# cgmb/euler

Measured on AMD Instinct MI355X. Metric: cells*steps/sec of sim_step() (frames incl. the PCG pressure projection) + pressure-solve HBM GB/s vs roofline, higher is better.
Workload: dtype f64

## Files before the change

### euler_amd/__init__.py

```python
import ctypes as C
import os

import numpy as np

_HERE = os.path.dirname(os.path.abspath(__file__))
LIB_PATH = os.path.join(_HERE, "lib", "libeuler_hip.so")

DOT_AUTO, DOT_SEQUENTIAL, DOT_TREE = 0, 1, 2
PRECOND_IC0, PRECOND_JACOBI, PRECOND_IC0_TILE, PRECOND_IC0_TILE2, PRECOND_IC0_TILE_MG = 0, 1, 2, 3, 4
(OPT_P_STEPS, OPT_TILE_STORE_AS, OPT_TILE_REVERSE, OPT_RESIDENT_CAP, OPT_GRID4_MIN_CELLS, OPT_SLAB_FUSION, OPT_RCCL_SMALL, OPT_RCCL_NO_EXCHANGE, OPT_MARKERS_ROWMAJOR,
 OPT_SA_RUN, OPT_NO_INTERIOR, OPT_BUILD_GATHER, OPT_RESIDENT_FORCE_TIMEOUT, OPT_MG_SPLIT_LEVEL, OPT_MG_SPLIT_ACTIVE, OPT_MARKERS_TWO_PASS, OPT_BUILD_TWO_PASS,
 OPT_VELOCITY_TWO_PASS, OPT_NO_TILE_MAP, OPT_PROFILE_STRIDE, OPT_TILE_STORE_Z, OPT_ADVECT_RK2, OPT_ADVECT_MACCORMACK) = range(1, 24)
SWEEP_AUTO, SWEEP_BAND, SWEEP_SIMPLE = 0, 1, 2
PCG_F64, PCG_F32 = 0, 1
RESIDENT_AUTO, RESIDENT_OFF = 0, 1
IMAGE_COVERAGE, IMAGE_DYE, IMAGE_SPEED = 0, 1, 2
EDIT_SOLID, EDIT_CLEAR, EDIT_SINK, EDIT_SOURCE, EDIT_FILL, EDIT_DRAIN = range(6)
OVERVIEW_DTYPE = np.dtype({"names": ["cells", "solid", "sink", "water", "marks", "max_speed2", "dye"],
                           "formats": [np.uint32, np.uint32, np.uint32, np.uint32, np.uint32, np.float32, (np.uint64, 3)],
                           "offsets": [0, 4, 8, 12, 16, 20, 24], "itemsize": 48})
DIAG_CROWDED = 8
DIAG_DTYPE = np.dtype({"names": ["cells", "fluid", "markers", "crowded", "mass_x", "mass_y", "div_l1", "ke_hi", "ke_lo", "count_max", "nonfinite", "max_div", "max_speed2"],
                       "formats": [np.uint64] * 9 + [np.uint32, np.uint32, np.float32, np.float32],
                       "offsets": [0, 8, 16, 24, 32, 40, 48, 56, 64, 72, 76, 80, 84], "itemsize": 88})
FLOW_PRESSURE = 1
PAINT_VORTICITY, PAINT_PRESSURE, PAINT_SPEED = 0, 1, 2
FLOW_DTYPE = np.dtype({"names": ["cells", "water", "nodes", "nonfinite", "u_pos", "u_neg", "v_pos", "v_neg", "w_pos", "w_neg", "p_sum", "max_speed2", "max_abs_w", "max_p", "reserved"],
                       "formats": [np.uint32] * 4 + [np.uint64] * 7 + [np.float32] * 3 + [np.uint32],
                       "offsets": [0, 4, 8, 12, 16, 24, 32, 40, 48, 56, 64, 72, 76, 80, 84], "itemsize": 88})
GAUGE_LEVEL, GAUGE_PRESSURE, GAUGE_FORCE, GAUGE_FLUX = range(4)
GAUGES_MAX = 1024
GAUGE_DTYPE = np.dtype({"names": ["kind", "x0", "y0", "x1", "y1", "reserved"], "formats": [np.int32] * 6, "offsets": [0, 4, 8, 12, 16, 20], "itemsize": 24})
GAUGE_REC_DTYPE = np.dtype({"names": ["cells", "fluid", "lo_x", "hi_x", "lo_y", "hi_y", "terms", "nonfinite", "a_pos", "a_neg", "b_pos", "b_neg", "max_a", "max_b"],
                            "formats": [np.uint32] * 8 + [np.uint64] * 4 + [np.float32] * 2,
                            "offsets": [0, 4, 8, 12, 16, 20, 24, 28, 32, 40, 48, 56, 64, 68], "itemsize": 72})
FORCE_BOXES_MAX = 64
FORCING_DTYPE = np.dtype({"names": ["gx", "gy", "shake_x", "shake_y", "shake_hz", "shake_phase", "nboxes", "reserved", "reserved2"],
                          "formats": [np.float32] * 4 + [np.float64] * 2 + [np.int32] * 2 + [np.float64],
                          "offsets": [0, 4, 8, 12, 16, 24, 32, 36, 40], "itemsize": 48})
FORCE_BOX_DTYPE = np.dtype({"names": ["x0", "y0", "x1", "y1", "fx", "fy"], "formats": [np.int32] * 4 + [np.float32] * 2, "offsets": [0, 4, 8, 12, 16, 20], "itemsize": 24})
HEAT_BOXES_MAX = 64
HEAT_FIX, HEAT_RATE = 0, 1
HEAT_DTYPE = np.dtype({"names": ["ambient", "beta", "kappa", "source_t", "nboxes", "reserved", "reserved2"],
                       "formats": [np.float32] * 4 + [np.int32] * 2 + [np.float64], "offsets": [0, 4, 8, 12, 16, 20, 24], "itemsize": 32})
HEAT_PX_DTYPE = np.dtype({"names": ["cells", "water", "t_pos", "t_neg", "max_above", "max_below"], "formats": [np.uint32] * 2 + [np.uint64] * 2 + [np.float32] * 2,
                          "offsets": [0, 4, 8, 16, 24, 28], "itemsize": 32})
HEAT_BOX_DTYPE = np.dtype({"names": ["x0", "y0", "x1", "y1", "value", "kind"], "formats": [np.int32] * 4 + [np.float32, np.int32], "offsets": [0, 4, 8, 12, 16, 20], "itemsize": 24})
BODIES_MAX = 16
BODY_DTYPE = np.dtype({"names": ["x", "y", "hz", "phase", "vx", "vy", "amp_x", "amp_y", "w", "h", "reserved"],
                       "formats": [np.float64] * 4 + [np.float32] * 4 + [np.int32] * 2 + [(np.int32, 2)],
                       "offsets": [0, 8, 16, 24, 32, 36, 40, 44, 48, 52, 56], "itemsize": 64})
BODY_STATE_DTYPE = np.dtype({"names": ["px", "py", "ox", "oy"], "formats": [np.float64] * 2 + [np.int32] * 2, "offsets": [0, 8, 16, 20], "itemsize": 24})
RESEED_DTYPE = np.dtype({"names": ["thin_above", "fill_holes", "max_cells", "max_fill", "reserved"], "formats": [np.int32] * 4 + [(np.int32, 4)],
                         "offsets": [0, 4, 8, 12, 16], "itemsize": 32})
RESEED_STATS_DTYPE = np.dtype({"names": ["removed", "added", "cells_thinned", "deferred"], "formats": [np.uint64] * 4, "offsets": [0, 8, 16, 24], "itemsize": 32})
ENV_ARRIVAL, ENV_WET, ENV_SPEED, ENV_PRESSURE, ENV_ALL = 1, 2, 4, 8, 15
ENV_NAMES = {ENV_ARRIVAL: "arrival", ENV_WET: "wet", ENV_SPEED: "speed", ENV_PRESSURE: "pressure"}
ENVELOPE_PX_DTYPE = np.dtype({"names": ["cells", "touched", "arrival_min", "arrival_max", "wet_max", "speed2_max", "p_max", "reserved"],
                              "formats": [np.uint32] * 8, "offsets": [0, 4, 8, 12, 16, 20, 24, 28], "itemsize": 32})
TRACERS_MAX = 1 << 22
TRACER_WET, TRACER_RETIRED, TRACER_IN_SOLID, TRACER_IN_SINK, TRACER_LOST, TRACER_WAS_DRY = 1, 2, 4, 8, 16, 32
TRACER_RASTER_ALL = 1
TRACER_DTYPE = np.dtype({"names": ["x", "y", "path", "age", "wet_time", "substeps", "flags", "reserved"],
                         "formats": [np.float32] * 5 + [np.uint32] * 3, "offsets": [0, 4, 8, 12, 16, 20, 24, 28], "itemsize": 32})
SESSION_IGNORE_SETTINGS = 1
SESSION_OPTS = 32
SESSION_SETTINGS_DTYPE = np.dtype({"names": ["max_iterations", "dot_mode", "precond", "tile_records", "sweep_mode", "max_substeps", "rainbow", "pcg_precision", "resident",
                                             "pcg_poll_interval", "viscosity_bits", "frame_time_bits", "tol", "nopts", "reserved", "opt"],
                                   "formats": [np.int32] * 10 + [np.uint32] * 2 + [np.float64] + [np.int32] * 2 + [(np.int64, SESSION_OPTS)],
                                   "offsets": [0, 4, 8, 12, 16, 20, 24, 28, 32, 36, 40, 44, 48, 56, 60, 64], "itemsize": 320})
SESSION_STAT_KEYS = ("last_substeps", "last_pcg_iterations", "last_residual", "last_dt", "pad", "marker_dt_events", "marker_multi_events")
SESSION_STAT_FORMAT = "<iidfIQQ"
SESSION_TAGS = (b"TIME", b"FORC", b"HEAT", b"TRAC", b"BODY", b"RSED", b"SETT", b"STAT", b"END\0")
GAUGE_VALUES = ("a", "b", "mean_a", "depth")
DIAG_VALUES = ("mean_abs_div", "kinetic_energy", "com_x", "com_y", "markers_per_cell", "crowded_fraction")
(F_U, F_V, F_UTMP, F_VTMP, F_SOLID, F_SOURCE, F_SINK, F_COUNT, F_PREV_COUNT, F_MARKERS, F_PRECON,
 F_PRESSURE, F_PCG_B, F_PCG_R, F_PCG_Z, F_PCG_S, F_PCG_Q, F_CELLMASK,
 F_DYE_R, F_DYE_G, F_DYE_B, F_DYE_RTMP, F_DYE_GTMP, F_DYE_BTMP, F_MARKER_KEYS) = range(25)
(STAGE_ADVECT_MARKERS, STAGE_REFRESH_COUNTS, STAGE_SOURCES, STAGE_EXTRAPOLATE, STAGE_ADVECT_VELOCITY,
 STAGE_PROJECT) = range(6)
(OP_BUILD_SYSTEM, OP_PRECON_FACTOR, OP_FORWARD_SOLVE, OP_BACKWARD_SOLVE, OP_APPLY_A, OP_DOT_ZR, OP_DOT_ZS,
 OP_INF_NORM_R, OP_UPDATE_PR, OP_UPDATE_SEARCH) = range(10)

_FIELD_DTYPE = {
    F_U: np.float32, F_V: np.float32, F_UTMP: np.float32, F_VTMP: np.float32,
    F_SOLID: np.uint8, F_SOURCE: np.uint8, F_SINK: np.uint8, F_COUNT: np.uint8, F_PREV_COUNT: np.uint8,
    F_MARKERS: np.float32, F_PRECON: np.float64, F_PRESSURE: np.float64, F_PCG_B: np.float64,
    F_PCG_R: np.float64, F_PCG_Z: np.float64, F_PCG_S: np.float64, F_PCG_Q: np.float64, F_CELLMASK: np.uint8,
    F_DYE_R: np.float32, F_DYE_G: np.float32, F_DYE_B: np.float32,
    F_DYE_RTMP: np.float32, F_DYE_GTMP: np.float32, F_DYE_BTMP: np.float32, F_MARKER_KEYS: np.uint32,
}


class EulerError(RuntimeError):
    def __init__(self, code, msg):
# ... 996 lines not shown
```

### euler_amd/csrc/driver.hip

```cpp
#include "euler_dev.h"
#include "k_mg.h"

#include <math.h>
#include <stdarg.h>
#include <stdlib.h>
#include <string.h>

#include <vector>

int eu_launch_build_system(euler_sim* S, float dt);
int eu_launch_velocity_update(euler_sim* S, float dt, int finish);
int eu_pressure_current(euler_sim* S);
int eu_unskew(euler_sim* S, const void* skew, void* rowmajor, int elem_bytes);
int eu_unskew_fluid(euler_sim* S, const double* skew, double* rowmajor);
double* eu_current_search_direction(euler_sim* S);
int eu_launch_tile_table(euler_sim* S);
int eu_skew(euler_sim* S, const void* rowmajor, void* skew, int elem_bytes);
int eu_set_source_count(euler_sim* S, size_t nsrc);

static thread_local char g_err[512] = "";

void eu_set_error(const char* fmt, ...) {
  va_list ap;
  va_start(ap, fmt);
// ... 56 lines not shown
}

extern "C" int euler_profile_class_count(void) { return KC__COUNT; }
extern "C" const char* euler_profile_class_name(int32_t c) { return (c >= 0 && c < KC__COUNT) ? k_class_names[c] : ""; }
extern "C" int euler_profile_enable(euler_sim* S, uint64_t mask) {
  if (!S) return EULER_EINVAL;
  int rc = eu_prof_flush(S);
  S->prof_mask = mask;
  S->prof_open = 0;
  return rc;
}
extern "C" int euler_profile_get(euler_sim* S, int32_t cls, double* ms, uint64_t* launches) {
  if (!S || cls < 0 || cls >= KC__COUNT) return EULER_EINVAL;
  int rc = eu_prof_flush(S);
  if (ms) *ms = S->prof_ms[cls];
  if (launches) *launches = S->prof_launches[cls];
  return rc;
}
extern "C" int euler_profile_reset(euler_sim* S) {
  if (!S) return EULER_EINVAL;
  int rc = eu_prof_flush(S);
  memset(S->prof_ms, 0, sizeof(S->prof_ms));
  memset(S->prof_launches, 0, sizeof(S->prof_launches));
  memset(S->prof_idle, 0, sizeof(S->prof_idle));
  return rc;
}

extern "C" int euler_config_default(euler_config* c) {
  if (!c) return EULER_EINVAL;
  memset(c, 0, sizeof(*c));
  c->abi_version = EULER_ABI_VERSION;
  c->X = 100; c->Y = 40;
  c->device = 0;
  c->max_iterations = 100;
  c->tol = (double)1e-6f;
  c->dot_mode = EULER_DOT_AUTO;
  c->precond = EULER_PRECOND_IC0;
  c->sweep_mode = EULER_SWEEP_AUTO;
  c->max_substeps = 8;
  c->frame_time = 0.1f;
  c->viscosity = 0.f;
  c->pcg_poll_interval = 8;
  return EULER_OK;
}

static int eu_set_tiles(euler_sim* S, int w) {
  if (w <= 0) w = 16;
  if (w != 8 && w != 16 && w != 32) { eu_set_error("precond_tile_records = %d: 8, 16 or 32 (0 = 16)", w); return EULER_EINVAL; }
  S->cfg.precond_tile_records = w;
  S->tile_w = w;
  return EULER_OK;
}

bool eu_resident_eligible(const euler_sim* S) {
  if (S->res_disabled || S->cfg.resident == EULER_RESIDENT_OFF) return false;
  if (S->cfg.precond != EULER_PRECOND_IC0_TILE || S->tile_w != 16 || S->cfg.sweep_mode == EULER_SWEEP_SIMPLE || S->cfg.dot_mode != EULER_DOT_TREE) return false;
  if (S->has_comm || S->slab_on || S->p2p_on) return false;
  const int cap = eu_resident_capacity(const_cast<euler_sim*>(S), S->cfg.pcg_precision == EULER_PCG_F32);
  if (S->cfg.pcg_precision == EULER_PCG_F32) return cap > 0 && S->geom.nbands * (S->geom.T / 16) <= 4 * cap;
  return cap > 0;
}
extern "C" int euler_resident_info(euler_sim* S, uint64_t out[3]) {
  if (!S || !out) return EULER_EINVAL;
  out[0] = eu_resident_eligible(S) ? 1 : 0; out[1] = S->res_solves; out[2] = S->res_fallbacks;
  return EULER_OK;
}

extern "C" int euler_set_option(euler_sim* S, int32_t key, int64_t value) {
  if (!S || key <= 0 || key >= EULER_OPT__COUNT) { eu_set_error("euler_set_option: unknown key %d", (int)key); return EULER_EINVAL; }
  bool ok = true;
  const char* when = nullptr;
  switch (key) {
    case EULER_OPT_P_STEPS: ok = value == 2 || value == 4 || value == 8; break;
    case EULER_OPT_SA_RUN: ok = value == 8 || value == 16 || value == 32;
      if (ok && value != 8 && (S->has_comm || eu_is_two_level(S))) when = "on a handle without a communicator, in the parity or the plain tile-local mode (the others run runs of 8)";
      break;
    case EULER_OPT_RCCL_SMALL: ok = value >= 0 && value <= 2; if (S->rccl) when = "before euler_set_comm_rccl"; break;
    case EULER_OPT_RCCL_NO_EXCHANGE: ok = value == 0 || value == 1; if (S->rccl) when = "before euler_set_comm_rccl"; break;
    case EULER_OPT_SLAB_FUSION: ok = value == 0 || value == 1; if (S->p2p_on) when = "before euler_p2p_connect"; break;
    case EULER_OPT_RESIDENT_CAP: case EULER_OPT_GRID4_MIN_CELLS: case EULER_OPT_RESIDENT_FORCE_TIMEOUT: ok = value >= 0; break;
    case EULER_OPT_MG_SPLIT_LEVEL: ok = value >= -1 && value < 12; break;
    case EULER_OPT_PROFILE_STRIDE: ok = value >= 1 && value <= 1024; break;
    case EULER_OPT_MG_SPLIT_ACTIVE: ok = false; break;
    case EULER_OPT_ADVECT_RK2: ok = value == 0 || value == 1;
      if (ok && value == 1 && S->slab_on) when = "on a whole-grid handle (row slabs: the midpoint samples reach one row beyond the ghost rows)";
      break;
    case EULER_OPT_ADVECT_MACCORMACK: ok = value == 0 || value == 1;
      if (ok && value == 1 && S->slab_on) when = "on a whole-grid handle (row slabs: the correction reads the forward result one row beyond the own rows)";
      break;
    default: ok = value == 0 || value == 1; break;
  }
  if (!ok) { eu_set_error("euler_set_option: key %d does not take the value %lld", (int)key, (long long)value); return EULER_EINVAL; }
  if (when) { eu_set_error("euler_set_option: key %d must be set %s", (int)key, when); return EULER_ESTATE; }
  HIPCHK(hipStreamSynchronize(S->stream));
  if (key == EULER_OPT_ADVECT_MACCORMACK && value == 1 && !S->mc_u) {
    float *a = nullptr, *b = nullptr;
    const size_t bytes = S->C * sizeof(float);
    if (eu_dalloc(S, &a, S->C, EU_MEM_HANDLE, EU_MEM_ZERO | EU_DEV_QUIET) || eu_dalloc(S, &b, S->C, EU_MEM_HANDLE, EU_MEM_ZERO | EU_DEV_QUIET)) {
      (void)eu_dev_free(S, a);
      eu_set_error("euler_set_option: EULER_OPT_ADVECT_MACCORMACK needs %zu bytes of scratch", 2 * bytes);
      return EULER_ENOMEM;
    }
    S->mc_u = a; S->mc_v = b;
  }
  if (key == EULER_OPT_P_STEPS || key == EULER_OPT_SA_RUN) {
    int rcp = eu_pressure_current(S);
    if (rcp) return rcp;
  }
  S->opt[key] = value;
  if (key == EULER_OPT_P_STEPS || key == EULER_OPT_SA_RUN) S->s_ring_n = 0;
  if (key == EULER_OPT_MG_SPLIT_LEVEL) { eu_mg_split_release(S); S->opt[EULER_OPT_MG_SPLIT_ACTIVE] = 0; }
  return EULER_OK;
}
extern "C" int euler_get_option(euler_sim* S, int32_t key, int64_t* value) {
  if (!S || !value || key <= 0 || key >= EULER_OPT__COUNT) { eu_set_error("euler_get_option: unknown key %d", (int)key); return EULER_EINVAL; }
  *value = S->opt[key];
  return EULER_OK;
}

static const char* eu_precond_combination(const euler_sim* S, int precond, int tile_w, int has_comm, int slab_on, int p2p_on) {
  const bool coarse = precond == EULER_PRECOND_IC0_TILE2 || precond == EULER_PRECOND_IC0_TILE_MG;
  if (!coarse) return nullptr;
  if (tile_w != 16 || S->cfg.sweep_mode == EULER_SWEEP_SIMPLE) return "the coarse-correction preconditioners run on tiles of 16 records with the band schedule";
  if (precond == EULER_PRECOND_IC0_TILE2 && (has_comm || slab_on)) return "EULER_PRECOND_IC0_TILE2 runs on one GPU (row slabs: EULER_PRECOND_IC0_TILE_MG)";
  if (precond == EULER_PRECOND_IC0_TILE_MG && has_comm && (!slab_on || p2p_on)) return "EULER_PRECOND_IC0_TILE_MG with several ranks: row-slab handles without mailboxes only";
  return nullptr;
}

extern "C" int euler_set_precond(euler_sim* S, int32_t precond, int32_t tile_records) {
  if (!S || precond < EULER_PRECOND_IC0 || precond > EULER_PRECOND_IC0_TILE_MG) { eu_set_error("euler_set_precond: bad argument"); return EULER_EINVAL; }
  const int w = tile_records <= 0 ? 16 : tile_records;
  if (w != 8 && w != 16 && w != 32) { eu_set_error("precond_tile_records = %d: 8, 16 or 32 (0 = 16)", tile_records); return EULER_EINVAL; }
  if (const char* why = eu_precond_combination(S, precond, w, S->has_comm, S->slab_on, S->p2p_on)) { eu_set_error("euler_set_precond: %s", why); return EULER_EINVAL; }
  if (S->cfg.pcg_precision == EULER_PCG_F32 && (precond != EULER_PRECOND_IC0_TILE || w != 16)) { eu_set_error("euler_set_precond: an EULER_PCG_F32 handle runs EULER_PRECOND_IC0_TILE with tiles of 16 records only"); return EULER_EINVAL; }
  HIPCHK(hipStreamSynchronize(S->stream));
  const bool coarse = precond == EULER_PRECOND_IC0_TILE2 || precond == EULER_PRECOND_IC0_TILE_MG;
  if (coarse) { int rc = eu_coarse_alloc(S, precond == EULER_PRECOND_IC0_TILE_MG); if (rc) return rc; }
  (void)eu_set_tiles(S, w);
  S->cfg.dot_mode = coarse ? EULER_DOT_TREE : S->dot_mode_user;
  if (S->has_comm && S->cfg.dot_mode == EULER_DOT_SEQUENTIAL) S->cfg.dot_mode = EULER_DOT_TREE;
  S->cfg.precond = precond;
  eu_vd_solver_arrays_foreign(&S->vd);
  return EULER_OK;
}

extern "C" int euler_set_solver(euler_sim* S, int32_t max_iterations, double tol) {
  if (!S) return EULER_EINVAL;
  HIPCHK(hipStreamSynchronize(S->stream));
  if (max_iterations > 0) S->cfg.max_iterations = max_iterations;
  if (tol >= 0.0) S->cfg.tol = tol;
  return EULER_OK;
}

#define DALLOC(p, n) do { int _rc = eu_dalloc(S, &(p), (n), EU_MEM_HANDLE, EU_MEM_ZERO); if (_rc) { euler_destroy(S); return _rc; } } while (0)

extern "C" void euler_destroy(euler_sim* S) {
  if (!S) return;
  if (S->stream) (void)hipStreamSynchronize(S->stream);
  eu_p2p_release(S);
  eu_rccl_release(S);
  eu_slab_release(S);
  eu_coarse_release(S);
  eu_dev_free_all(S);
  if (S->ms_host) (void)hipHostFree(S->ms_host);
  if (S->sc_host) (void)hipHostFree(S->sc_host);
  if (S->poll_host) (void)hipHostFree(S->poll_host);
// ... 849 lines not shown
```

### euler_amd/csrc/euler_dev.h

```cpp
#pragma once

#include <hip/hip_runtime.h>
#include <stdint.h>
#include <stdio.h>

#include "euler.h"
#include "euler_host.h"
#include "eu_valid.h"
#include "eu_mem.h"

#define EU_H 1.0f
#define EU_RHO 1.0f
#define EU_G (-10.0f)

#define CM_FLUID 0x01
#define CM_RIGHT 0x02
#define CM_UP    0x04
#define CM_LEFT  0x08
#define CM_DOWN  0x10
#define CM_DIAG_SHIFT 5
#define CM_INTERIOR 0x9F
#define EU_CHUNK_INTERIOR 0x80000000u

enum {
  KC_TIMESTEP = 0, KC_MARKER_ADVECT, KC_MARKER_EVENTS, KC_MARKER_BIN, KC_MARKER_COMPACT, KC_SOURCES,
  KC_SELECT, KC_EXTRAPOLATE, KC_ADVECT_VELOCITY, KC_BUILD_SYSTEM, KC_PRECON_FACTOR,
  KC_FORWARD_SOLVE, KC_BACKWARD_SOLVE, KC_APPLY_A, KC_DOT, KC_UPDATE_PR, KC_UPDATE_SEARCH,
  KC_REDUCE_FINAL, KC_VELOCITY_UPDATE, KC_JACOBI, KC_MISC, KC_PRECOND_TILE, KC_COARSE_CYCLE, KC_RESIDENT, KC__COUNT
};

struct PcgScalars {
  double sigma, zs, sigma_new, alpha, beta, rnorm;
  double tol;
  double comm_val;
  double comm_val2;
  double* comm_slot;
  double alpha_prev;
  double alpha_hist[8];
  int nonzero;
  int done;
  int iters;
  int max_iters;
  unsigned int n_chunks;
  unsigned int zfix;
  void** p2p_boxes;
  int* p2p_error;
  int p2p_rank, p2p_n;
  unsigned int p2p_seq, p2p_halo_seq;
};

struct MarkerState {
  unsigned long long n;
  unsigned long long max_markers;
  unsigned long long rng_state;
  int exhausted;
  unsigned int n_events;
  unsigned int n_actual;
  unsigned int n_deleted;
  unsigned int n_append;
  unsigned long long n0_append;
  unsigned long long total_dt_events, multi_events;
  float dt_final;
  float dt;
  unsigned int max_u2_bits, max_v2_bits;
  unsigned int dt_ticket;
  int error;
  unsigned long long n_loc;
  unsigned int n_rm;
  unsigned int n_del_glob;
  unsigned int n_recv;
  unsigned int src_k_lo;
  unsigned long long rng0;
  unsigned int rs_crowded;
  unsigned int rs_k;
  unsigned int rs_holes;
  unsigned int rs_fill;
  unsigned long long rs_n0;
  unsigned long long rs_rng0;
  unsigned long long rs_removed, rs_added, rs_thinned, rs_deferred;
};

#define EU_SKEW_SLACK (64 * 64)
#ifndef EU_ARRAY_STAGGER
#define EU_ARRAY_STAGGER 0
#endif
#ifndef EU_RED_ELEMS
#define EU_RED_ELEMS (256 * 16)
#endif
struct SkewGeom {
  int X, Y, nbands, T, TS;
  size_t S;
};
static inline __host__ __device__ size_t skew_index(const SkewGeom& g, int x, int y) {
  const int l = y & 63, t = x + l;
  return ((size_t)(y >> 6) * g.TS + (size_t)(t & ~1)) * 64 + 2 * l + (t & 1);
}
static inline __host__ __device__ void skew_decode(const SkewGeom& g, size_t e, int& band, int& t, int& l) {
  const size_t per_band = (size_t)g.TS * 64;
  band = (int)(e / per_band);
  const size_t r = e % per_band;
  l = (int)((r & 127) >> 1);
  t = (int)((r >> 7) << 1) + (int)(r & 1);
}

struct SelectScratch {
  unsigned int* block_sums;
  unsigned int* total;
  size_t capacity_blocks;
};

struct eu_devbuf { void* p; size_t bytes; };

struct euler_sim {
  euler_config cfg;
  int X, Y;
  size_t C;
  hipStream_t stream;
  int loaded;
  long long opt[32];
  int dot_mode_user;

  float *u, *v, *utmp, *vtmp;
  uint8_t *solid, *source, *sink, *count, *prev_count;
  unsigned int* count32;
  eu_valid vd;
  unsigned long long* delmask;
  uint8_t* tmap;
// ... 13 lines not shown
  size_t n_tracers;
  euler_heat heat;
  euler_heat_box heat_boxes[EULER_HEAT_BOXES_MAX];
  int heat_on, heat_cur;
  int heat_ghost_stale;
  unsigned int heat_ntiles;
  eu_devbuf heat_buf, heat_box_buf, heat_fill_buf, heat_ras_buf;
  int n_bodies;
  euler_body bodies[EULER_BODIES_MAX];
  int32_t body_ox[EULER_BODIES_MAX], body_oy[EULER_BODIES_MAX];
  euler_reseed reseed;
  int reseed_on;
  eu_devbuf rs_mask_buf, rs_cell_buf, rs_slot_buf, rs_draw_buf;
  uint32_t env_channels;
  uint64_t env_substeps;
  uint32_t* env_plane[4];
  eu_devbuf env_ras_buf;
  float *mc_u, *mc_v;
  float2* markers[2];
  int cur;
  size_t max_markers;
  unsigned long long n_markers_host;
  size_t n_source_cells;
  MarkerState* ms;
  MarkerState* ms_host;
  unsigned long long* evmask;
  float* ev_theta;
  float* ev_delta;
  unsigned int* sel_idx;
  size_t sel_cap;
  unsigned int* act_idx; float* act_dt;
  unsigned long long* cellmask64;
  float* draws;
  SelectScratch sel;

  SkewGeom geom;
  double *b, *p, *r, *z, *s, *q, *precon;
  double* s2;
  uint8_t* cellmask;
  uint8_t* sys_m; float* sys_div;
  unsigned int* fbits_fwd; unsigned int* fbits_bwd;
  int fb_stride;
  int4* band_ranges;
  int coarse_m, coarse_shift, coarse_nx, coarse_ny, coarse_n;
  int *cc_diag, *cc_right, *cc_up;
  int* cc_pinned;
  double* cc_sten;
  int cc_n;
  double* cc_fac;
  double* cc_inv;
  double* cc_part;
  double* cc_y;
  double* cc_null;
  int mg_levels, mg_nx[12], mg_ny[12];
  size_t mg_off[12], mg_cells;
  double* mg_a;
  unsigned long long* mg_a0i;
  double *mg_rhs, *mg_x;
  double* mg_wd;
  uint8_t* mg_inner0; double mg_ic[9];
  double* mg_part;
  double* mg_dot;
  double* mg_null0;
  double* mg_m0;
  void* mg_split;
  double* mg_xbuf; int mg_xslot;
  unsigned long long* res_gran;
  unsigned long long res_tag;
  int* res_err;
  int res_disabled;
  unsigned int res_last_chunks;
  int res_have_last, res_skip_once;
  unsigned long long res_solves, res_fallbacks;
  int pcg_fields_resident;
  int tile_w;
  double* s_ring[8];
  void* s_ring_alloc[8];
  double* s_base[2];
  int s_ring_n;
  int s_launched;
  int s_none;
  int s_stale;
  const double* tile_as_override;
  double* partial2;
  struct RngJump* rng_jump;
  uint8_t* chunk_flag;
  uint8_t* chunk_prev;
  uint8_t* chunk_part;
  eu_mem mem;
  double* zhalo;
  double* zrows;
  int z_halo_last;
  double* tile_table;
  unsigned long long* chunk_bits;
  unsigned int* chunk_list;
  size_t chunk_words, chunk_cap;
  double* xrows;
  size_t xrow_len;
  int gs_cur;
  double* alpha_buf;
  double* pair_buf;
  double* rowmajor_tmp;
  PcgScalars* sc;
  PcgScalars* sc_host;
  PcgScalars* poll_host;
  hipEvent_t poll_event[2];
  double* partial;
  unsigned int* red_counter;
  int red_blocks;
  unsigned long long* granules;
  int gran_stride;
  unsigned int* ticket;
  unsigned int ticket_base;
  unsigned int epoch;
  unsigned long long* sweep_timeline;

  float interp_lim[4];

  euler_stats stats;

  euler_comm_ops comm;
  int has_comm, couple;
  int band_lo, band_hi;
  size_t e_lo, e_cnt;
  double* halo_buf;
  int own_stream;
  int slab_on;
  int row_lo, row_hi, win_lo, win_hi;
  size_t win_off, Cw, skew_off, Sw;
  int ab_lo, ab_hi;
  unsigned int* keys[2];
  euler_comm_ops bulk;
  struct SlabScratch* slab;
  int part_lo[64], part_hi[64];
  void* rccl;
  void* p2p;
  int p2p_on;

  uint64_t prof_mask;
  uint64_t prof_open;
  unsigned int prof_seq[32];
  double prof_ms[KC__COUNT];
  uint64_t prof_launches[KC__COUNT];
  uint64_t prof_idle[KC__COUNT];
  hipEvent_t* ev_pool; int* ev_cls; int* ev_solve; int* ev_iter; int ev_used, ev_cap;
  int solve_seq;
  int prof_iter;
  int solve_iters[256];
};

void eu_set_error(const char* fmt, ...);
int eu_hip_fail(hipError_t e, const char* what, const char* file, int line);
#define HIPCHK(call) do { hipError_t _e = (call); if (_e != hipSuccess) return eu_hip_fail(_e, #call, __FILE__, __LINE__); } while (0)

void eu_prof_begin(euler_sim* S, int cls);
void eu_prof_end(euler_sim* S, int cls);
int  eu_prof_flush(euler_sim* S);

#define LAUNCH(S, CLS, KERNEL, GRID, BLOCK, ...)                                   \
  do {                                                                             \
    eu_prof_begin((S), (CLS));                                                     \
    hipLaunchKernelGGL(KERNEL, GRID, BLOCK, 0, (S)->stream, __VA_ARGS__);          \
    eu_prof_end((S), (CLS));                                                       \
  } while (0)

static inline unsigned eu_blocks(size_t n, unsigned per_block, unsigned cap = 0x7fffffffu) {
  size_t b = (n + per_block - 1) / per_block;
  if (b < 1) b = 1;
  if (b > cap) b = cap;
  return (unsigned)b;
}

__device__ __forceinline__ size_t eu_xcd_block() {
  const unsigned int b = blockIdx.x, full = gridDim.x & ~7u;
  return b < full ? (size_t)(b & 7) * (full >> 3) + (b >> 3) : (size_t)b;
// ... 236 lines not shown
```

### euler_amd/csrc/k_grid.hip

```cpp
#include "k_pcg.h"
#include "k_transport.h"

#include <stdlib.h>

__device__ __forceinline__ void dt_from_maxima(MarkerState* ms, float frame_time_left, unsigned int mu_bits, unsigned int mv_bits) {
  const float mu = __uint_as_float(mu_bits), mv = __uint_as_float(mv_bits);
  const float max_distance = 0.75f * EU_H;
  const float max_velocity = sqrtf(mu + mv);
  ms->dt = fminf(max_distance / max_velocity, frame_time_left);
  ms->max_u2_bits = 0u;
  ms->max_v2_bits = 0u;
}
template <bool FUSE_DT>
__global__ __launch_bounds__(256) void k_maxsq(const float* __restrict__ u, const float* __restrict__ v,
                                               int X, int Y, MarkerState* ms, int y0, int y1, float frame_time_left) {
  float mu = 0.f, mv = 0.f;
  const bool vec = (X & 3) == 0;
  for (int yq = y0 + 4 * (int)blockIdx.x; yq < y1; yq += 4 * (int)gridDim.x) {
    if (vec) {
      for (int x = 4 * (int)threadIdx.x; x < X; x += 4 * 256) {
        float4 a[4], b[4];
#pragma unroll
        for (int r = 0; r < 4; ++r) {
          const int y = yq + r < y1 ? yq + r : y1 - 1;
// ... 591 lines not shown
      sm[ll[k]][jj[k]] = mm[k];
      sd[ll[k]][jj[k]] = dv[k];
      if (mm[k] & CM_FLUID) s_fl[jj[k] / 16] = 1;
      if (mm[k] != CM_INTERIOR) s_part[jj[k] / 16] = 1;
    }
  }
  __syncthreads();
  const float k_inv_scale_f = (EU_H * EU_H) * EU_RHO / dt;
  bool nz = false;
  for (int c = tid; c < 64 * BS_W; c += 256) {
    const int pr = c >> 7, l = (c & 127) >> 1, j = 2 * pr + (c & 1);
    const int ch = j / 16;
    const bool touch = s_fl[ch] || s_prev[ch];
    const int x = t0 + j - l, y = band * 64 + l;
    if (!touch || x < 0 || x >= X || y >= Y) continue;
    const uint8_t m = sm[l][j];
    const double bv = m ? -(double)sd[l][j] * (double)k_inv_scale_f : 0.0;
    nz = nz || bv != 0.0;
    const size_t e = ((size_t)band * g.TS + (size_t)(t0 + 2 * pr)) * 64 + (size_t)(c & 127);
    cellmask[e] = m;
    b[e] = bv;
    r[e] = bv;
    p[e] = 0.0;
    if (!TILE) { q[e] = 0.0; z[e] = 0.0; }
  }
  if (nz) s_nz = 1;
  __syncthreads();
  if (tid < BS_W / 16) {
    if (s_fl[tid]) chunk_flag[chunk0 + tid] = 1;
    if (s_part[tid]) chunk_part[chunk0 + tid] = 1;
  }
  if (tid == 0 && s_nz && __hip_atomic_load(&sc->nonzero, __ATOMIC_RELAXED, __HIP_MEMORY_SCOPE_AGENT) == 0) atomicOr(&sc->nonzero, 1);
}

__global__ __launch_bounds__(256) void k_pack_chunk_bits(const uint8_t* __restrict__ flag, unsigned long long* __restrict__ bits, size_t nwords, size_t nchunks) {
  const size_t w = (size_t)blockIdx.x * blockDim.x + threadIdx.x;
  if (w >= nwords) return;
  unsigned long long v = 0;
  for (int k = 0; k < 64; ++k) {
    const size_t c = w * 64 + k;
    if (c < nchunks && flag[c]) v |= 1ull << k;
  }
  bits[w] = v;
}

__global__ __launch_bounds__(256) void k_velocity_update(const float* __restrict__ uin, const float* __restrict__ vin,
                                                         float* __restrict__ uout, float* __restrict__ vout,
                                                         double* p, const uint8_t* __restrict__ count,
                                                         const uint8_t* __restrict__ solid, SkewGeom g, float dt, int y0, int y1) {
  const int X = g.X, Y = g.Y;
  const int x = blockIdx.x * 64 + (threadIdx.x & 63);
  const int y = y0 + blockIdx.y * 4 + (threadIdx.x >> 6);
  if (x >= X || y >= y1) return;
  const size_t i = (size_t)y * X + x;
  const size_t e = skew_index(g, x, y);
  const bool f0 = count[i] != 0;
  double p0 = p[e];
  if (f0 && p0 < 0.0) { p0 = 0.0; p[e] = 0.0; }
  const float neg_inv = -(1.f / (EU_RHO * EU_H));
  if (x < X - 1) {
    const bool f1 = count[i + 1] != 0;
    float o = 0.f;
    if (solid[i] | solid[i + 1]) o = 0.f;
    else if (f0 | f1) {
      double p1 = p[skew_index(g, x + 1, y)];
      if (f1 && p1 < 0.0) p1 = 0.0;
      o = uin[i] + (neg_inv * (float)(p1 - p0)) * dt;
    }
    uout[i] = o;
  }
  if (y < Y - 1) {
    const bool f1 = count[i + X] != 0;
    float o = 0.f;
    if (solid[i] | solid[i + X]) o = 0.f;
    else if (f0 | f1) {
      double p1 = p[skew_index(g, x, y + 1)];
      if (f1 && p1 < 0.0) p1 = 0.0;
      o = vin[i] + (neg_inv * (float)(p1 - p0)) * dt;
    }
    vout[i] = o;
  }
}

struct VuRing { const double* s[8]; int n, steps, use; };
#define VU_W 48
#define VU_ILP 4
__global__ __launch_bounds__(256) void k_velocity_update_para(const float* __restrict__ uin, const float* __restrict__ vin, float* __restrict__ uout, float* __restrict__ vout,
                                                              const double* __restrict__ p, const uint8_t* __restrict__ mask, const uint8_t* __restrict__ count,
                                                              const uint8_t* __restrict__ solid, SkewGeom g, float dt, const PcgScalars* sc, VuRing ring, MarkerState* ms,
                                                              int band_lo, int do_max, int skip_zero,
                                                              const uint8_t* __restrict__ tmap, int tnx) {
  __shared__ double sp[65][VU_W + 1];
  __shared__ float s_mu[4], s_mv[4];
  const int units = g.T / VU_W;
  const size_t blk = eu_xcd_block();
  const int band = band_lo + (int)(blk / units), t0 = (int)(blk % units) * VU_W;
  const int X = g.X, Y = g.Y, tid = threadIdx.x;
  if (skip_zero && tmap && eu_tiles_idle_cur(tmap, tnx, band, t0 > 63 ? (t0 - 63) >> 6 : 0, (t0 + VU_W - 1) >> 6, true)) return;
  int cnt = 0, from = 0;
  if (ring.use && sc->nonzero && sc->iters > 0) {
    const int n_it = sc->iters;
    from = n_it - 1 >= ring.steps ? (n_it - 1) / ring.steps * ring.steps : 0;
    cnt = n_it - from;
  }
  double al[8];
  const double* sq[8];
#pragma unroll
  for (int j = 0; j < 8; ++j) { const int it = from + (j < cnt ? j : 0); al[j] = sc->alpha_hist[it & 7]; sq[j] = ring.s[it % ring.n]; }
  const size_t ebase = ((size_t)band * g.TS + (size_t)t0) * 64;
  static_assert((64 * VU_W) % (256 * VU_ILP) == 0, "whole rounds of VU_ILP elements per thread");
  for (int c0 = tid; c0 < 64 * VU_W; c0 += 256 * VU_ILP) {
    uint8_t m[VU_ILP];
    double pv[VU_ILP];
    bool any = false;
#pragma unroll
    for (int u = 0; u < VU_ILP; ++u) { m[u] = mask[ebase + (size_t)(c0 + 256 * u)]; any = any || (m[u] & CM_FLUID); }
    if (__any(any)) {
#pragma unroll
      for (int u = 0; u < VU_ILP; ++u) pv[u] = p[ebase + (size_t)(c0 + 256 * u)];
#pragma unroll
      for (int j = 0; j < 8; ++j)
        if (j < cnt) {
          double sv[VU_ILP];
#pragma unroll
          for (int u = 0; u < VU_ILP; ++u) sv[u] = sq[j][ebase + (size_t)(c0 + 256 * u)];
#pragma unroll
          for (int u = 0; u < VU_ILP; ++u) pv[u] = pv[u] + sv[u] * al[j];
        }
    } else {
#pragma unroll
      for (int u = 0; u < VU_ILP; ++u) pv[u] = 0.0;
    }
#pragma unroll
    for (int u = 0; u < VU_ILP; ++u) {
      const int c = c0 + 256 * u;
      const double v = (m[u] & CM_FLUID) ? (pv[u] < 0.0 ? 0.0 : pv[u]) : 0.0;
      sp[(c & 127) >> 1][2 * (c >> 7) + (c & 1)] = v;
    }
  }
  {
    size_t e = 0;
    bool want = false, above = false;
    int hl = 0, hj = 0;
    if (tid < 64) { e = ebase + (size_t)VU_W * 64 + 2 * (size_t)tid; want = true; hl = tid; hj = VU_W; }
    else if (tid < 64 + VU_W) {
      const int j = tid - 64 + 1, x = t0 - 64 + j;
      hl = 64; hj = j;
      if (x >= 0 && x < X && band + 1 < g.nbands && count[(size_t)(band + 1) * 64 * X + x] != 0) { e = ((size_t)(band + 1) * g.TS + (size_t)(x & ~1)) * 64 + (size_t)(x & 1); want = true; above = true; }
    }
    if (tid < 64 + VU_W) {
      double pv = 0.0;
      if (want && (above || (mask[e] & CM_FLUID))) {
        pv = p[e];
#pragma unroll
        for (int j = 0; j < 8; ++j) if (j < cnt) pv = pv + sq[j][e] * al[j];
        pv = pv < 0.0 ? 0.0 : pv;
      }
      sp[hl][hj] = pv;
    }
  }
  __syncthreads();
  const float neg_inv = -(1.f / (EU_RHO * EU_H));
  float mu = 0.f, mv = 0.f;
  static_assert((64 * VU_W) % (256 * 4) == 0, "whole rounds of four cells per thread");
  for (int c0 = tid; c0 < 64 * VU_W; c0 += 256 * 4) {
    size_t ii[4]; bool in[4]; int ll[4], jj[4], xx[4], yy[4];
    uint8_t c_0[4], c_r[4], c_u[4], s_0[4], s_r[4], s_u[4];
    float ui[4], vi[4];
#pragma unroll
    for (int u = 0; u < 4; ++u) {
      const int c = c0 + 256 * u;
      ll[u] = c / VU_W; jj[u] = c % VU_W;
      xx[u] = t0 - ll[u] + jj[u]; yy[u] = band * 64 + ll[u];
      in[u] = xx[u] >= 0 && xx[u] < X && yy[u] < Y;
      ii[u] = (size_t)(yy[u] < Y ? yy[u] : Y - 1) * X + (size_t)(xx[u] < 0 ? 0 : xx[u] >= X ? X - 1 : xx[u]);
      const bool hr = in[u] && xx[u] < X - 1, hu = in[u] && yy[u] < Y - 1;
      c_0[u] = count[ii[u]]; s_0[u] = solid[ii[u]];
      c_r[u] = count[ii[u] + (hr ? 1 : 0)]; s_r[u] = solid[ii[u] + (hr ? 1 : 0)];
      c_u[u] = count[ii[u] + (hu ? (size_t)X : (size_t)0)]; s_u[u] = solid[ii[u] + (hu ? (size_t)X : (size_t)0)];
    }
    bool wet = false;
#pragma unroll
    for (int u = 0; u < 4; ++u) wet = wet || ((c_0[u] | c_r[u] | c_u[u]) != 0);
    if (__any(wet)) {
#pragma unroll
      for (int u = 0; u < 4; ++u) { ui[u] = uin[ii[u]]; vi[u] = vin[ii[u]]; }
// ... 23 lines not shown
        if (s_0[u] | s_u[u]) o = 0.f;
        else if (f0 | f1) { o = vi[u] + (neg_inv * (float)(sp[l + 1][j + 1] - p0)) * dt; live = true; }
        if (live || !skip_zero) vout[ii[u]] = o;
        const float sqv = o * o; if (sqv > mv) mv = sqv;
      }
    }
  }
  mu = eu_wave_maxf(mu);
  mv = eu_wave_maxf(mv);
  if ((tid & 63) == 0) { s_mu[tid >> 6] = mu; s_mv[tid >> 6] = mv; }
  __syncthreads();
  if (tid == 0 && do_max) {
    for (int k = 1; k < 4; ++k) { if (s_mu[k] > mu) mu = s_mu[k]; if (s_mv[k] > mv) mv = s_mv[k]; }
    if (mu > 0.f) atomicMax(&ms->max_u2_bits, __float_as_uint(mu));
    if (mv > 0.f) atomicMax(&ms->max_v2_bits, __float_as_uint(mv));
  }
}
__global__ __launch_bounds__(256) void k_clamp_p(double* __restrict__ p, const uint8_t* __restrict__ mask, size_t e_lo, size_t S) {
  for (size_t i = e_lo + (size_t)blockIdx.x * blockDim.x + threadIdx.x; i < e_lo + S; i += (size_t)gridDim.x * blockDim.x)
    if ((mask[i] & CM_FLUID) && p[i] < 0.0) p[i] = 0.0;
}

__global__ __launch_bounds__(256) void k_mark_interior(unsigned int* __restrict__ list, const PcgScalars* sc, const uint8_t* __restrict__ part) {
  const unsigned int i = blockIdx.x * blockDim.x + threadIdx.x;
  if (i >= sc->n_chunks) return;
  const unsigned int c = list[i];
  if (!part[c]) list[i] = c | EU_CHUNK_INTERIOR;
}

int eu_launch_build_system(euler_sim* S, float dt) {
  uint8_t* t = S->chunk_flag; S->chunk_flag = S->chunk_prev; S->chunk_prev = t;
  HIPCHK(hipMemsetAsync(S->chunk_flag, 0, S->chunk_cap + 64, S->stream));
  HIPCHK(hipMemsetAsync(S->chunk_part, 0, S->chunk_cap + 64, S->stream));
  const bool lean = eu_vd_lean_assembly(&S->vd, eu_is_tile(S) && S->cfg.sweep_mode != EULER_SWEEP_SIMPLE);
  const bool gather = S->opt[EULER_OPT_BUILD_GATHER] != 0;
  const bool two_pass = S->opt[EULER_OPT_BUILD_TWO_PASS] != 0;
  if (!gather && !two_pass) {
    const unsigned nblk = (unsigned)((size_t)(S->band_hi - S->band_lo) * (S->geom.T / BS_W));
    if (lean)
      LAUNCH(S, KC_BUILD_SYSTEM, k_build_system_para<true>, dim3(nblk), dim3(256), S->utmp, S->vtmp, S->count, S->solid, S->b, S->r, S->p, S->q, S->z, S->cellmask, S->sc, S->geom, dt, S->band_lo,
             S->chunk_flag, S->chunk_part, S->chunk_prev, eu_tile_map_on(S) ? (const uint8_t*)S->tmap : (const uint8_t*)nullptr, S->tmap_nx);
    else
      LAUNCH(S, KC_BUILD_SYSTEM, k_build_system_para<false>, dim3(nblk), dim3(256), S->utmp, S->vtmp, S->count, S->solid, S->b, S->r, S->p, S->q, S->z, S->cellmask, S->sc, S->geom, dt, S->band_lo,
             S->chunk_flag, S->chunk_part, S->chunk_prev, (const uint8_t*)nullptr, 0);
  } else if (!gather) {
    const size_t win_off = (size_t)S->win_lo * S->X;
    LAUNCH(S, KC_BUILD_SYSTEM, k_cell_system, dim3(eu_blocks((size_t)S->X * (S->row_hi - S->row_lo), 256)), dim3(256), S->utmp, S->vtmp, S->count, S->solid, S->sys_m, S->sys_div,
           S->X, S->row_lo, S->row_hi, win_off);
    if (lean)
      LAUNCH(S, KC_BUILD_SYSTEM, k_build_system2<true>, dim3(eu_blocks(S->e_cnt, 256)), dim3(256), S->sys_m, S->sys_div, win_off, S->b, S->r, S->p, S->q, S->z, S->cellmask, S->sc,
             S->geom, dt, S->e_lo, S->e_cnt, S->chunk_flag, S->chunk_part, S->chunk_prev);
    else
      LAUNCH(S, KC_BUILD_SYSTEM, k_build_system2<false>, dim3(eu_blocks(S->e_cnt, 256)), dim3(256), S->sys_m, S->sys_div, win_off, S->b, S->r, S->p, S->q, S->z, S->cellmask, S->sc,
             S->geom, dt, S->e_lo, S->e_cnt, S->chunk_flag, S->chunk_part, S->chunk_prev);
  } else if (lean)
    LAUNCH(S, KC_BUILD_SYSTEM, k_build_system<true>, dim3(eu_blocks(S->e_cnt, 256)), dim3(256), S->utmp, S->vtmp, S->count,
           S->solid, S->b, S->r, S->p, S->q, S->z, S->cellmask, S->sc, S->geom, dt, S->e_lo, S->e_cnt, S->chunk_flag, S->chunk_part, S->chunk_prev);
  else
    LAUNCH(S, KC_BUILD_SYSTEM, k_build_system<false>, dim3(eu_blocks(S->e_cnt, 256)), dim3(256), S->utmp, S->vtmp, S->count,
           S->solid, S->b, S->r, S->p, S->q, S->z, S->cellmask, S->sc, S->geom, dt, S->e_lo, S->e_cnt, S->chunk_flag, S->chunk_part, S->chunk_prev);
  eu_vd_assembled(&S->vd);
  LAUNCH(S, KC_BUILD_SYSTEM, k_pack_chunk_bits, dim3(eu_blocks(S->chunk_words, 256)), dim3(256), S->chunk_flag, S->chunk_bits, S->chunk_words, S->chunk_cap);
  int rc = eu_ordered_select(S, S->chunk_bits, S->chunk_words, S->chunk_list, &S->sc->n_chunks);
  if (rc) return rc;
  const bool no_interior = S->opt[EULER_OPT_NO_INTERIOR] != 0;
  if (!no_interior)
    LAUNCH(S, KC_BUILD_SYSTEM, k_mark_interior, dim3(eu_blocks(S->chunk_cap, 256)), dim3(256), S->chunk_list, S->sc, S->chunk_part);
  return eu_launch_band_ranges(S);
}

int eu_pressure_current(euler_sim* S) {
  const int mode = eu_vd_pressure_owes(&S->vd);
  if (!mode) return EULER_OK;
  eu_vd_pressure_made_current(&S->vd);
  if (mode == 1) { int rc = eu_launch_finish_p(S); if (rc) return rc; }
  LAUNCH(S, KC_VELOCITY_UPDATE, k_clamp_p, dim3(eu_blocks(S->e_cnt, 256 * 4, 4096)), dim3(256), S->p, S->cellmask, S->e_lo, S->e_cnt);
  return EULER_OK;
}
int eu_launch_velocity_update(euler_sim* S, float dt, int finish) {
  const bool one_pass = (!S->has_comm || S->slab_on) && S->opt[EULER_OPT_VELOCITY_TWO_PASS] == 0 && (!S->slab_on || !finish);
  if (one_pass) {
    VuRing ring;
    for (int k = 0; k < 8; ++k) ring.s[k] = S->s_ring[k < S->s_ring_n ? k : 0];
    ring.n = S->s_ring_n > 0 ? S->s_ring_n : 1; ring.steps = ring.n; ring.use = finish && S->s_ring_n > 0;
    if (!ring.use) for (int k = 0; k < 8; ++k) ring.s[k] = S->p;
    const int do_max = S->slab_on ? 0 : 1;
    if (eu_vd_update_clears_maxima(&S->vd, do_max)) HIPCHK(hipMemsetAsync(&S->ms->max_u2_bits, 0, 2 * sizeof(unsigned int), S->stream));
    LAUNCH(S, KC_VELOCITY_UPDATE, k_velocity_update_para, dim3((unsigned)((size_t)(S->band_hi - S->band_lo) * (S->geom.T / VU_W))), dim3(256), S->utmp, S->vtmp, S->u, S->v, S->p, S->cellmask,
           S->count, S->solid, S->geom, dt, S->sc, ring, S->ms, S->band_lo, do_max, eu_vd_update_skips_zeros(&S->vd, S->slab_on),
           eu_tile_map_on(S) ? (const uint8_t*)S->tmap : (const uint8_t*)nullptr, S->tmap_nx);
    eu_vd_velocity_updated(&S->vd, 1, ring.use, do_max);
    return EULER_OK;
  }
  if (finish) { int rc = eu_launch_finish_p(S); if (rc) return rc; }
  dim3 grid((S->X + 63) / 64, (S->row_hi - S->row_lo + 3) / 4);
  LAUNCH(S, KC_VELOCITY_UPDATE, k_velocity_update, grid, dim3(256), S->utmp, S->vtmp, S->u, S->v, S->p, S->count,
         S->solid, S->geom, dt, S->row_lo, S->row_hi);
  eu_vd_velocity_updated(&S->vd, 0, 0, 0);
  return EULER_OK;
}

template <typename T>
__global__ __launch_bounds__(256) void k_unskew(const T* __restrict__ skew, T* __restrict__ rowmajor, SkewGeom g, int y0, int y1) {
  const size_t i = (size_t)blockIdx.x * blockDim.x + threadIdx.x;
  if (i < (size_t)g.X * (y1 - y0)) rowmajor[i] = skew[skew_index(g, (int)(i % g.X), y0 + (int)(i / g.X))];
}
template <typename T>
__global__ __launch_bounds__(256) void k_skew(const T* __restrict__ rowmajor, T* __restrict__ skew, SkewGeom g, int y0, int y1) {
  const size_t i = (size_t)blockIdx.x * blockDim.x + threadIdx.x;
  if (i < (size_t)g.X * (y1 - y0)) skew[skew_index(g, (int)(i % g.X), y0 + (int)(i / g.X))] = rowmajor[i];
}

__global__ __launch_bounds__(256) void k_unskew_fluid(const double* __restrict__ skew, const uint8_t* __restrict__ mask, double* __restrict__ rowmajor, SkewGeom g, int y0, int y1) {
  const size_t i = (size_t)blockIdx.x * blockDim.x + threadIdx.x;
  if (i >= (size_t)g.X * (y1 - y0)) return;
  const size_t e = skew_index(g, (int)(i % g.X), y0 + (int)(i / g.X));
  rowmajor[i] = (mask[e] & CM_FLUID) ? skew[e] : 0.0;
}
int eu_unskew_fluid(euler_sim* S, const double* skew, double* rowmajor) {
  const unsigned nb = eu_blocks((size_t)S->X * (S->row_hi - S->row_lo), 256);
  hipLaunchKernelGGL(k_unskew_fluid, dim3(nb), dim3(256), 0, S->stream, skew, S->cellmask, rowmajor, S->geom, S->row_lo, S->row_hi);
  return EULER_OK;
}
int eu_unskew(euler_sim* S, const void* skew, void* rowmajor, int elem_bytes) {
  const unsigned nb = eu_blocks((size_t)S->X * (S->row_hi - S->row_lo), 256);
  if (elem_bytes == 8) hipLaunchKernelGGL(k_unskew<double>, dim3(nb), dim3(256), 0, S->stream, (const double*)skew, (double*)rowmajor, S->geom, S->row_lo, S->row_hi);
  else hipLaunchKernelGGL(k_unskew<uint8_t>, dim3(nb), dim3(256), 0, S->stream, (const uint8_t*)skew, (uint8_t*)rowmajor, S->geom, S->row_lo, S->row_hi);
  return EULER_OK;
}
int eu_skew(euler_sim* S, const void* rowmajor, void* skew, int elem_bytes) {
  const unsigned nb = eu_blocks((size_t)S->X * (S->row_hi - S->row_lo), 256);
  if (elem_bytes == 8) hipLaunchKernelGGL(k_skew<double>, dim3(nb), dim3(256), 0, S->stream, (const double*)rowmajor, (double*)skew, S->geom, S->row_lo, S->row_hi);
  else hipLaunchKernelGGL(k_skew<uint8_t>, dim3(nb), dim3(256), 0, S->stream, (const uint8_t*)rowmajor, (uint8_t*)skew, S->geom, S->row_lo, S->row_hi);
  return EULER_OK;
}
```

### euler_amd/csrc/k_pcg.h

```cpp
#pragma once

#include "euler_dev.h"
#include "k_mg.h"

#define COMM_CALL(expr) do { if ((expr) != 0) { eu_set_error("communicator callback failed: %s", #expr); return EULER_ECOMM; } } while (0)
#define LOC(ptr) ((ptr) + S->e_lo)
enum { SW_FACTOR = 0, SW_FORWARD = 1, SW_BACKWARD = 2 };

int eu_launch_build_system(euler_sim* S, float dt);
int eu_launch_velocity_update(euler_sim* S, float dt, int finish);
int eu_launch_band_ranges(euler_sim* S);
int eu_launch_sweep(euler_sim* S, int op, int cls, int force, int fin_qq = -1);
int eu_launch_factor_tile(euler_sim* S, int force);
int eu_launch_precond_tile(euler_sim* S, int rupd, int sweeps, int fin_dot, int force, double alpha, bool r_only = false, int zform = -1);
int eu_launch_search_apply(euler_sim* S, int it);
int eu_launch_finish_p(euler_sim* S);
int eu_launch_dot(euler_sim* S, const double* a, const double* b, int fin_op, int force);
int eu_comm_exchange(euler_sim* S, double* send_lo, double* send_hi, double* recv_lo, double* recv_hi, int count, double* small, int nsmall);
int eu_comm_finish(euler_sim* S, int fin_op, int is_max, int force);
int eu_comm_halo_two(euler_sim* S, double* a, double* b);
bool tile_recompute(const euler_sim* S);
int p_steps(const euler_sim* S);

enum { FIN_SIGMA_INIT = 0, FIN_ALPHA, FIN_RNORM, FIN_BETA, FIN_STORE_ONLY, FIN_TO_COMM };
#define FIN_VIA_P2P 0x100

static inline bool tile_fused(const euler_sim* S) { return eu_is_tile(S) && S->cfg.sweep_mode != EULER_SWEEP_SIMPLE; }
static inline bool ghost_mode(const euler_sim* S) { return S->has_comm && !S->p2p_on && tile_fused(S); }
enum { XR_ZSEND_LO = 0, XR_ZSEND_HI, XR_ZRECV_LO, XR_ZRECV_HI, XR_GS_LO0, XR_GS_LO1, XR_GS_HI0, XR_GS_HI1 };
static inline double* xrow(const euler_sim* S, int k) { return S->xrows + (size_t)k * S->xrow_len; }
static inline int sa_run(const euler_sim* S) {
  if (S->opt[EULER_OPT_SA_RUN] != 8 && !S->has_comm && !eu_is_two_level(S)) return (int)S->opt[EULER_OPT_SA_RUN];
  return 8;
}
static inline bool tile_z_recompute(const euler_sim* S) {
  return tile_recompute(S) && tile_fused(S) && !eu_is_two_level(S) && S->tile_w == 16 && !S->has_comm && !S->slab_on && S->band_lo == 0 &&
         S->opt[EULER_OPT_TILE_STORE_Z] == 0 && S->chunk_list && S->tile_table;
}
static inline int fin_or_comm(const euler_sim* S, int fin_op) {
  return S->has_comm ? (S->p2p_on ? (fin_op | FIN_VIA_P2P) : (int)FIN_TO_COMM) : fin_op;
}

#ifdef __HIPCC__
#define RED_THREADS 1024
typedef double sw_d2 __attribute__((ext_vector_type(2)));

__device__ __forceinline__ bool pcg_idle(const PcgScalars* sc) { return sc->done || !sc->nonzero; }

#define DPP_WAVE_SHL1 0x130
#define DPP_WAVE_SHR1 0x138

template <int CTRL>
__device__ __forceinline__ double wave_shift_inject(double v, double edge) {
  const int lo = __builtin_amdgcn_update_dpp(__double2loint(edge), __double2loint(v), CTRL, 0xf, 0xf, false);
  const int hi = __builtin_amdgcn_update_dpp(__double2hiint(edge), __double2hiint(v), CTRL, 0xf, 0xf, false);
  return __hiloint2double(hi, lo);
}


__device__ __forceinline__ void pcg_scalar_step(PcgScalars* sc, int op, double v) {
  switch (op) {
    case FIN_SIGMA_INIT: sc->sigma = v; break;
    case FIN_ALPHA: sc->zs = v; sc->alpha_prev = sc->alpha; sc->alpha = sc->sigma / v; sc->alpha_hist[sc->iters & 7] = sc->alpha; sc->iters += 1; break;
    case FIN_RNORM: sc->rnorm = v; if (v <= sc->tol) sc->done = 1; break;
    case FIN_BETA: sc->sigma_new = v; sc->beta = v / sc->sigma; sc->sigma = v; break;
    case FIN_TO_COMM: sc->comm_val = v; if (sc->comm_slot) *sc->comm_slot = v; break;
    default: sc->sigma_new = v; break;
  }
}

template <int NT = RED_THREADS>
__device__ __forceinline__ double block_sum(double v) {
  __shared__ double sw[NT / 64];
  v = eu_wave_sum(v);
  __syncthreads();
  if ((threadIdx.x & 63) == 0) sw[threadIdx.x >> 6] = v;
  __syncthreads();
  double t = 0.0;
  if (threadIdx.x == 0) for (int k = 0; k < NT / 64; ++k) t += sw[k];
  return t;
}
template <int NT = RED_THREADS>
__device__ __forceinline__ double block_max(double v) {
  __shared__ double sm[NT / 64];
  v = eu_wave_max(v);
  __syncthreads();
  if ((threadIdx.x & 63) == 0) sm[threadIdx.x >> 6] = v;
  __syncthreads();
  double t = 0.0;
  if (threadIdx.x == 0) for (int k = 0; k < NT / 64; ++k) t = sm[k] > t ? sm[k] : t;
  return t;
}

template <bool IS_MAX, int NT = RED_THREADS>
__device__ __forceinline__ void block_finish(double v_block, double* partial, unsigned int* counter, PcgScalars* sc, int op) {
  __shared__ int am_last;
  if (threadIdx.x == 0) {
    __hip_atomic_store(reinterpret_cast<unsigned long long*>(&partial[blockIdx.x]),
                       (unsigned long long)__double_as_longlong(v_block), __ATOMIC_RELAXED, __HIP_MEMORY_SCOPE_AGENT);
    asm volatile("s_waitcnt vmcnt(0)" ::: "memory");
    const unsigned int t = __hip_atomic_fetch_add(counter, 1u, __ATOMIC_RELAXED, __HIP_MEMORY_SCOPE_AGENT);
    am_last = t == gridDim.x - 1;
  }
  __syncthreads();
  if (!am_last) return;
  double v = 0.0;
  for (unsigned int i = threadIdx.x; i < gridDim.x; i += NT) {
    const double w = __longlong_as_double((long long)__hip_atomic_load(
        reinterpret_cast<unsigned long long*>(&partial[i]), __ATOMIC_RELAXED, __HIP_MEMORY_SCOPE_AGENT));
    if (IS_MAX) v = w > v ? w : v; else v += w;
  }
  v = IS_MAX ? block_max<NT>(v) : block_sum<NT>(v);
  if (op & FIN_VIA_P2P) { v = p2p_allreduce_block<IS_MAX>(sc, v); op &= 0xff; }
  if (threadIdx.x == 0) {
    pcg_scalar_step(sc, op, v);
    __hip_atomic_store(counter, 0u, __ATOMIC_RELAXED, __HIP_MEMORY_SCOPE_AGENT);
  }
}

__device__ __forceinline__ void st_system(const double* p, double v) {
// ... 30 lines not shown
    const double res = (cm & CM_FLUID) ? qv : 0.0;
    const double carry = -1.0 * cpre * res;
    own = carry; out = carry;
    if (j & 1) zz[j >> 1].y = res; else zz[j >> 1].x = res;
  }
  own = 0.0; out = 0.0;
#pragma unroll
  for (int j = W - 1; j >= 0; --j) {
    const int cm = (int)((mm[j >> 1] >> ((j & 1) * 8)) & 0xff);
    const double cin = (j & 1) ? zz[j >> 1].y : zz[j >> 1].x, cpre = (j & 1) ? pp[j >> 1].y : pp[j >> 1].x;
    const double nbv = wave_shift_inject<DPP_WAVE_SHL1>(out, 0.0);
    const double kr = ((cm & CM_RIGHT) ? -1.0 : 0.0) * cpre, ku = ((cm & CM_UP) ? -1.0 : 0.0) * cpre;
    const double t = cin - kr * own - ku * nbv;
    const double zv = t * cpre;
    const double res = (cm & CM_FLUID) ? zv : 0.0;
    own = res; out = res;
    if (DOT && (cm & CM_FLUID)) dsum += res * ((j & 1) ? rr[j >> 1].y : rr[j >> 1].x);
    if (j & 1) zz[j >> 1].y = res; else zz[j >> 1].x = res;
  }
}
struct ZrArgs { const double* r; const double* pre; const double* table; const double* halo; const double* rows; int X; };
struct CoarseRef { const double* y; int shift, nx, ny, band0; };
struct SaHist { const double* s[6]; };

struct SweepArgs {
  SkewGeom g;
  const uint8_t* mask;
  const unsigned int* fbits_fwd;
  const unsigned int* fbits_bwd;
  int fb_stride;
  double* pre;
  const double* in;
  double* out;
  unsigned long long* granules;
  int gran_stride;
  const unsigned long long* xg_in;
  unsigned long long* xg_out;
  const int4* ranges;
  int band_lo, nb_local;
  int couple;
  unsigned int* ticket;
  unsigned int ticket_base;
  unsigned int epoch;
  const PcgScalars* sc;
  int force;
  int* error;
  unsigned long long* timeline;
  int tile_w;
  int fin_qq;
  double* qq_partial;
  unsigned int* qq_counter;
  PcgScalars* sc_w;
};

struct TileArgs {
  SkewGeom g;
  const uint8_t* mask;
  double* pre;
  double* r;
  const double* as;
  double* z;
  int band_lo, nb_local;
  int rupd;
  int sweeps;
  int fin_dot;
  int via;
  double* part_max; double* part_dot;
  unsigned int* counter;
  const unsigned int* list;
  const double* table;
  PcgScalars* sc;
  int force;
  double alpha_arg;
  double* pair_slot;
  double *zsend_lo, *zsend_hi;
  int edge_lo, edge_hi;
  int reverse;
  double* cpart;
  int cshift;
  int cmode, cnx, cny;
  const double *gs_lo, *gs_hi;
  int zform;
  double *zhalo, *zrows;
};

__device__ __forceinline__ double factor_step(double aa, double own, double nbv) {
  const double cl = -1.0 * own, cb = -1.0 * nbv;
  double e = aa - cl * cl - cb * cb;
  if (e < 0.25 * aa) e = (aa != 0.0) ? aa : 1.0;
  return 1.0 / sqrt(e);
}

template <int CTRL>
__device__ __forceinline__ double dpp_move(double v) {
  const int lo = __builtin_amdgcn_update_dpp(0, __double2loint(v), CTRL, 0xf, 0xf, true);
  const int hi = __builtin_amdgcn_update_dpp(0, __double2hiint(v), CTRL, 0xf, 0xf, true);
  return __hiloint2double(hi, lo);
}
__device__ __forceinline__ double group_sum(double v) {
  v = v + dpp_move<0xB1>(v);
  v = v + dpp_move<0x4E>(v);
  if (MG_LG == 8) v = v + dpp_move<0x141>(v);
  return v;
}
#endif
```

### euler_amd/csrc/k_pcg.hip

```cpp
#include "k_pcg.h"

#include <cmath>
#include <vector>

template <bool IS_MAX>
__global__ __launch_bounds__(RED_THREADS) void k_reduce_final(const double* __restrict__ partial, int n, PcgScalars* sc,
                                                              int op, int force) {
  if (!force && pcg_idle(sc)) return;
  double v = 0.0;
  for (int i = threadIdx.x; i < n; i += RED_THREADS) {
    const double w = partial[i];
    if (IS_MAX) v = w > v ? w : v; else v += w;
  }
  v = IS_MAX ? block_max(v) : block_sum(v);
  if (threadIdx.x == 0) pcg_scalar_step(sc, op, v);
}

template <bool EDGES>
__global__ __launch_bounds__(RED_THREADS) void k_dot_partial(const double* __restrict__ a, const double* __restrict__ b,
                                                             const uint8_t* __restrict__ mask, size_t S,
                                                             double* __restrict__ partial, PcgScalars* sc, int force,
                                                             unsigned int* counter, int fin_op, int TS, int nb_local, int edges) {
  if (!force && pcg_idle(sc)) return;
  const size_t chunk = (((S + gridDim.x - 1) / gridDim.x) + 1) & ~(size_t)1;
  const size_t lo = (size_t)blockIdx.x * chunk, hi = lo + chunk < S ? lo + chunk : S;
  double t = 0.0;
  for (size_t i = lo + 2 * (size_t)threadIdx.x; i < hi; i += 2 * RED_THREADS) {
    const unsigned int mm = *reinterpret_cast<const unsigned short*>(mask + i);
    if (!((mm | (mm >> 8)) & CM_FLUID)) continue;
    const sw_d2 av = *reinterpret_cast<const sw_d2*>(a + i), bv = *reinterpret_cast<const sw_d2*>(b + i);
    if (mm & CM_FLUID) t += av.x * bv.x;
    if ((mm >> 8) & CM_FLUID) t += av.y * bv.y;
    if (EDGES && slab_edge_row(i, (int)((i & 127) >> 1), TS, nb_local, edges)) {
      if (mm & CM_FLUID) st_system(a + i, av.x);
      if ((mm >> 8) & CM_FLUID) st_system(a + i + 1, av.y);
    }
  }
  if (EDGES) asm volatile("s_waitcnt vmcnt(0)" ::: "memory");
  t = block_sum(t);
  block_finish<false>(t, partial, counter, sc, fin_op);
}

#define SEQ_TILE 4096
__global__ __launch_bounds__(256) void k_dot_sequential(const double* __restrict__ a, const double* __restrict__ b,
                                                        const uint8_t* __restrict__ mask, SkewGeom g, PcgScalars* sc,
                                                        int op, int force) {
  if (!force && pcg_idle(sc)) return;
  __shared__ double prod[2][SEQ_TILE];
  __shared__ unsigned long long any[2][SEQ_TILE / 64];
  const size_t C = (size_t)g.X * g.Y;
  const int ntiles = (int)((C + SEQ_TILE - 1) / SEQ_TILE);
  const int wave = threadIdx.x >> 6, lane = threadIdx.x & 63;
  double total = 0.0;
  for (int tile = -1; tile < ntiles; ++tile) {
    if (wave > 0 && tile + 1 < ntiles) {
      const int buf = (tile + 1) & 1;
      const size_t base = (size_t)(tile + 1) * SEQ_TILE;
      for (int grp = wave - 1; grp < SEQ_TILE / 64; grp += 3) {
        const size_t c = base + (size_t)grp * 64 + lane;
        bool f = false;
        double pr = 0.0;
        if (c < C) {
          const size_t i = skew_index(g, (int)(c % g.X), (int)(c / g.X));
          f = (mask[i] & CM_FLUID) != 0;
          if (f) pr = a[i] * b[i];
        }
        prod[buf][grp * 64 + lane] = pr;
        const unsigned long long bal = __ballot(f);
        if (lane == 0) any[buf][grp] = bal;
      }
    }
    if (threadIdx.x == 0 && tile >= 0) {
      const int buf = tile & 1;
      for (int grp = 0; grp < SEQ_TILE / 64; ++grp) {
        if (any[buf][grp] == 0ull) continue;
        const double* pp = &prod[buf][grp * 64];
        double v[64];
#pragma unroll
        for (int k = 0; k < 64; ++k) v[k] = pp[k];
#pragma unroll
        for (int k = 0; k < 64; ++k) total += v[k];
      }
    }
    __syncthreads();
  }
  if (threadIdx.x == 0) pcg_scalar_step(sc, op, total);
}

__global__ __launch_bounds__(RED_THREADS) void k_apply_a(const double* __restrict__ s, double* __restrict__ z,
                                                         const uint8_t* __restrict__ mask, SkewGeom g,
                                                         double* __restrict__ partial, PcgScalars* sc, int force,
                                                         unsigned int* counter, int fin_op) {
  if (!force && pcg_idle(sc)) return;
  const size_t S = g.S;
  const size_t chunk = (((S + gridDim.x - 1) / gridDim.x) + 127) & ~(size_t)127;
  const size_t lo = (size_t)blockIdx.x * chunk, hi = lo + chunk < S ? lo + chunk : S;
  double t = 0.0;
  for (size_t i = lo + 2 * (size_t)threadIdx.x; i < hi; i += 2 * RED_THREADS) {
    const unsigned int mm = *reinterpret_cast<const unsigned short*>(mask + i);
    const unsigned int m0 = mm & 0xff, m1 = mm >> 8;
    if (!((m0 | m1) & CM_FLUID)) continue;
    const sw_d2 c = *reinterpret_cast<const sw_d2*>(s + i);
    const int l = (int)((i & 127) >> 1);
    sw_d2 o = {0.0, 0.0};
    if (m0 & CM_FLUID) {
      double v = (double)(int)(m0 >> CM_DIAG_SHIFT) * c.x;
      v = v - ((m0 & CM_RIGHT) ? c.y : 0.0);
      if (m0 & CM_UP) {
        size_t up = i + 3;
        if (l == 63) { int band, tt, ll; skew_decode(g, i, band, tt, ll); up = skew_index(g, tt - 63, 64 * (band + 1)); }
        v = v - s[up];
      } else {
        v = v - 0.0;
      }
      v = v - ((m0 & CM_LEFT) ? s[i - 127] : 0.0);
      if (m0 & CM_DOWN) {
        size_t dn = i - 129;
        if (l == 0) { int band, tt, ll; skew_decode(g, i, band, tt, ll); dn = skew_index(g, tt, 64 * band - 1); }
        v = v - s[dn];
      } else {
        v = v - 0.0;
      }
      o.x = v;
      t += v * c.x;
    }
    if (m1 & CM_FLUID) {
      double v = (double)(int)(m1 >> CM_DIAG_SHIFT) * c.y;
      v = v - ((m1 & CM_RIGHT) ? s[i + 128] : 0.0);
      if (m1 & CM_UP) {
        size_t up = i + 130;
        if (l == 63) { int band, tt, ll; skew_decode(g, i + 1, band, tt, ll); up = skew_index(g, tt - 63, 64 * (band + 1)); }
        v = v - s[up];
      } else {
        v = v - 0.0;
      }
      v = v - ((m1 & CM_LEFT) ? c.x : 0.0);
      if (m1 & CM_DOWN) {
        size_t dn = i - 2;
        if (l == 0) { int band, tt, ll; skew_decode(g, i + 1, band, tt, ll); dn = skew_index(g, tt, 64 * band - 1); }
        v = v - s[dn];
      } else {
        v = v - 0.0;
      }
      o.y = v;
      t += v * c.y;
    }
    if ((m0 & m1) & CM_FLUID) *reinterpret_cast<sw_d2*>(z + i) = o;
    else if (m0 & CM_FLUID) z[i] = o.x;
    else z[i + 1] = o.y;
  }
  t = block_sum(t);
  if (fin_op >= 0) block_finish<false>(t, partial, counter, sc, fin_op);
}

__global__ __launch_bounds__(RED_THREADS) void k_update_pr(double* __restrict__ p, double* __restrict__ r,
                                                           const double* __restrict__ s, const double* __restrict__ z,
                                                           const uint8_t* __restrict__ mask, size_t S,
                                                           double* __restrict__ partial, PcgScalars* sc, int force,
                                                           double alpha_arg, unsigned int* counter, int fin_op) {
  if (!force && pcg_idle(sc)) return;
  const double alpha = force ? alpha_arg : sc->alpha;
  const double nalpha = -alpha;
  const size_t chunk = (((S + gridDim.x - 1) / gridDim.x) + 1) & ~(size_t)1;
  const size_t lo = (size_t)blockIdx.x * chunk, hi = lo + chunk < S ? lo + chunk : S;
  double mx = 0.0;
  for (size_t i = lo + 2 * (size_t)threadIdx.x; i < hi; i += 2 * RED_THREADS) {
    const unsigned int mm = *reinterpret_cast<const unsigned short*>(mask + i);
    const bool f0 = (mm & CM_FLUID) != 0, f1 = ((mm >> 8) & CM_FLUID) != 0;
    if (!(f0 | f1)) continue;
    const sw_d2 sv = *reinterpret_cast<const sw_d2*>(s + i), zv = *reinterpret_cast<const sw_d2*>(z + i);
    sw_d2 pv = *reinterpret_cast<const sw_d2*>(p + i), rv = *reinterpret_cast<const sw_d2*>(r + i);
    if (f0) { pv.x = pv.x + sv.x * alpha; rv.x = rv.x + zv.x * nalpha; const double a = fabs(rv.x); if (a > mx) mx = a; }
    if (f1) { pv.y = pv.y + sv.y * alpha; rv.y = rv.y + zv.y * nalpha; const double a = fabs(rv.y); if (a > mx) mx = a; }
    *reinterpret_cast<sw_d2*>(p + i) = pv;
    *reinterpret_cast<sw_d2*>(r + i) = rv;
  }
  mx = block_max(mx);
  if (fin_op >= 0) block_finish<true>(mx, partial, counter, sc, fin_op);
}

__global__ __launch_bounds__(RED_THREADS) void k_inf_norm(const double* __restrict__ r, const uint8_t* __restrict__ mask,
                                                          size_t S, double* __restrict__ partial) {
  const size_t chunk = (S + gridDim.x - 1) / gridDim.x;
  const size_t lo = (size_t)blockIdx.x * chunk, hi = lo + chunk < S ? lo + chunk : S;
  double mx = 0.0;
  for (size_t i = lo + threadIdx.x; i < hi; i += RED_THREADS)
    if (mask[i] & CM_FLUID) { const double a = fabs(r[i]); if (a > mx) mx = a; }
  mx = block_max(mx);
  if (threadIdx.x == 0) partial[blockIdx.x] = mx;
}

template <bool COPY>
__global__ __launch_bounds__(256) void k_update_search(double* __restrict__ s, const double* __restrict__ z,
                                                       const uint8_t* __restrict__ mask, size_t S, const PcgScalars* sc,
                                                       int force, double beta_arg) {
  if (!force && pcg_idle(sc)) return;
  const double beta = force ? beta_arg : sc->beta;
  for (size_t i = 2 * ((size_t)blockIdx.x * blockDim.x + threadIdx.x); i < S; i += 2 * (size_t)gridDim.x * blockDim.x) {
    const sw_d2 zv = *reinterpret_cast<const sw_d2*>(z + i);
    if (COPY) { *reinterpret_cast<sw_d2*>(s + i) = zv; continue; }
    const unsigned int mm = *reinterpret_cast<const unsigned short*>(mask + i);
    const bool f0 = (mm & CM_FLUID) != 0, f1 = ((mm >> 8) & CM_FLUID) != 0;
    if (!(f0 | f1)) continue;
    sw_d2 sv = *reinterpret_cast<const sw_d2*>(s + i);
    if (f0) sv.x = zv.x + beta * sv.x;
    if (f1) sv.y = zv.y + beta * sv.y;
    *reinterpret_cast<sw_d2*>(s + i) = sv;
  }
}

__global__ __launch_bounds__(256) void k_publish_edge_rows(double* arr, SkewGeom g, int y0, int y1, const PcgScalars* sc) {
  if (pcg_idle(sc)) return;
  const int x = blockIdx.x * 256 + threadIdx.x;
  if (x >= g.X) return;
  const int y = blockIdx.y == 0 ? y0 : y1;
  if (y < 0) return;
  double* p = arr + skew_index(g, x, y);
  st_system(p, *p);
}

__global__ __launch_bounds__(256) void k_jacobi(const double* __restrict__ r, double* __restrict__ z,
                                                const uint8_t* __restrict__ mask, size_t S, const PcgScalars* sc, int force) {
  if (!force && pcg_idle(sc)) return;
  for (size_t i = (size_t)blockIdx.x * blockDim.x + threadIdx.x; i < S; i += (size_t)gridDim.x * blockDim.x) {
    const uint8_t m = mask[i];
    const int d = m >> CM_DIAG_SHIFT;
    z[i] = (m & CM_FLUID) ? r[i] / (double)(d ? d : 1) : 0.0;
  }
}

struct SRing { const double* s[8]; int n, steps; };
__global__ __launch_bounds__(256) void k_finish_p(double* __restrict__ p, const uint8_t* __restrict__ mask, size_t e_lo, size_t S,
                                                  const PcgScalars* sc, SRing ring) {
  if (!sc->nonzero || sc->iters == 0) return;
  const int n_it = sc->iters;
  const int from = n_it - 1 >= ring.steps ? (n_it - 1) / ring.steps * ring.steps : 0;
  const int cnt = n_it - from;
  double al[8];
  const double* sp[8];
#pragma unroll
  for (int j = 0; j < 8; ++j) { const int it = from + (j < cnt ? j : 0); al[j] = sc->alpha_hist[it & 7]; sp[j] = ring.s[it % ring.n] + e_lo; }
  for (size_t i = 2 * ((size_t)blockIdx.x * blockDim.x + threadIdx.x); i < S; i += 2 * (size_t)gridDim.x * blockDim.x) {
    const unsigned int mm = *reinterpret_cast<const unsigned short*>(mask + i);
    const bool f0 = (mm & CM_FLUID) != 0, f1 = ((mm >> 8) & CM_FLUID) != 0;
    if (!(f0 | f1)) continue;
    sw_d2 pv = *reinterpret_cast<const sw_d2*>(p + i);
#pragma unroll
    for (int j = 0; j < 8; ++j) {
      if (j < cnt) {
        const sw_d2 sv = *reinterpret_cast<const sw_d2*>(sp[j] + i);
        if (f0) pv.x = pv.x + sv.x * al[j];
        if (f1) pv.y = pv.y + sv.y * al[j];
      }
    }
    *reinterpret_cast<sw_d2*>(p + i) = pv;
  }
}

int eu_launch_finish_p(euler_sim* S) {
  if (S->s_ring_n <= 0) return EULER_OK;
  SRing ring;
  for (int k = 0; k < 8; ++k) ring.s[k] = S->s_ring[k < S->s_ring_n ? k : 0];
  ring.n = S->s_ring_n; ring.steps = S->s_ring_n;
  LAUNCH(S, KC_UPDATE_PR, k_finish_p, dim3(eu_blocks(S->e_cnt, 256 * 4, 4096)), dim3(256), S->p + S->e_lo, S->cellmask + S->e_lo, S->e_lo, S->e_cnt, S->sc, ring);
  return EULER_OK;
}

__global__ void k_scalar_epilogue(PcgScalars* sc, int op, int force) {
  if (!force && pcg_idle(sc)) return;
  pcg_scalar_step(sc, op, sc->comm_val);
}
__global__ void k_nonzero_to_comm(PcgScalars* sc) { sc->comm_val = sc->nonzero ? 1.0 : 0.0; }
__global__ void k_nonzero_from_comm(PcgScalars* sc) { sc->nonzero = sc->comm_val != 0.0; }

__global__ __launch_bounds__(256) void k_pack_row(const double* __restrict__ skew, double* __restrict__ row, SkewGeom g, int band, int lane) {
  const int x = blockIdx.x * 256 + threadIdx.x;
  if (x < g.X) row[x] = skew[skew_index(g, x, band * 64 + lane)];
}
__global__ __launch_bounds__(256) void k_unpack_row(double* __restrict__ skew, const double* __restrict__ row, SkewGeom g, int band, int lane) {
  const int x = blockIdx.x * 256 + threadIdx.x;
  if (x < g.X) skew[skew_index(g, x, band * 64 + lane)] = row[x];
}

template <bool PACK>
__global__ __launch_bounds__(256) void k_halo_rows2(double* a, double* b, double* lo, double* hi, SkewGeom g, int band_lo, int band_hi,
                                                    int has_lo, int has_hi) {
  const int x = blockIdx.x * 256 + threadIdx.x;
  if (x >= g.X) return;
  const int side = blockIdx.y >> 1, vec = blockIdx.y & 1;
  if (side == 0 ? !has_lo : !has_hi) return;
  double* arr = vec ? b : a;
  double* buf = (side ? hi : lo) + (size_t)vec * g.X;
  const int y = PACK ? (side ? 64 * band_hi - 1 : 64 * band_lo) : (side ? 64 * band_hi : 64 * band_lo - 1);
  double* e = arr + skew_index(g, x, y);
  if (PACK) buf[x] = *e; else *e = buf[x];
}

int eu_comm_exchange(euler_sim* S, double* send_lo, double* send_hi, double* recv_lo, double* recv_hi, int count, double* small, int nsmall) {
  if (S->bulk.exchange) {
    COMM_CALL(S->bulk.exchange(S->bulk.ctx, send_lo, send_hi, recv_lo, recv_hi, count, small, nsmall));
    return EULER_OK;
  }
  if (count > 0) COMM_CALL(S->bulk.halo(S->bulk.ctx, send_lo, send_hi, recv_lo, recv_hi, count));
  if (nsmall > 0) {
    int64_t off[64], cnt[64];
    for (int r = 0; r < S->bulk.nranks && r < 64; ++r) { off[r] = (int64_t)8 * nsmall * r; cnt[r] = (int64_t)8 * nsmall; }
    COMM_CALL(S->bulk.allgather(S->bulk.ctx, small, off, cnt));
  }
  return EULER_OK;
}
__global__ void k_alpha_fold(PcgScalars* sc, const double* __restrict__ vals, int R, int force) {
  if (!force && pcg_idle(sc)) return;
  double v = 0.0;
  for (int r = 0; r < R; ++r) v += vals[r];
  pcg_scalar_step(sc, FIN_ALPHA, v);
}

int eu_comm_finish(euler_sim* S, int fin_op, int is_max, int force) {
  if (S->p2p_on) return EULER_OK;
  if (fin_op == FIN_ALPHA && ghost_mode(S)) {
    if (int rc = eu_comm_exchange(S, nullptr, nullptr, nullptr, nullptr, 0, S->alpha_buf, 1)) return rc;
    hipLaunchKernelGGL(k_alpha_fold, dim3(1), dim3(1), 0, S->stream, S->sc, S->alpha_buf, S->comm.nranks, force);
    return EULER_OK;
  }
  COMM_CALL(S->comm.allreduce(S->comm.ctx, &S->sc->comm_val, 1, is_max));
  hipLaunchKernelGGL(k_scalar_epilogue, dim3(1), dim3(1), 0, S->stream, S->sc, fin_op, force);
  return EULER_OK;
}

static int comm_halo_s(euler_sim* S) {
  if (S->p2p_on) return eu_p2p_halo_skewed(S, S->s);
  const int X = S->X, nbk = (X + 255) / 256;
  double *send_lo = S->halo_buf, *send_hi = S->halo_buf + X, *recv_lo = S->halo_buf + 2 * X, *recv_hi = S->halo_buf + 3 * X;
  const bool has_lo = S->band_lo > 0, has_hi = S->band_hi < S->geom.nbands;
  if (has_lo) hipLaunchKernelGGL(k_pack_row, dim3(nbk), dim3(256), 0, S->stream, S->s, send_lo, S->geom, S->band_lo, 0);
  if (has_hi) hipLaunchKernelGGL(k_pack_row, dim3(nbk), dim3(256), 0, S->stream, S->s, send_hi, S->geom, S->band_hi - 1, 63);
  COMM_CALL(S->comm.halo(S->comm.ctx, send_lo, send_hi, recv_lo, recv_hi, X));
  if (has_lo) hipLaunchKernelGGL(k_unpack_row, dim3(nbk), dim3(256), 0, S->stream, S->s, recv_lo, S->geom, S->band_lo - 1, 63);
  if (has_hi) hipLaunchKernelGGL(k_unpack_row, dim3(nbk), dim3(256), 0, S->stream, S->s, recv_hi, S->geom, S->band_hi, 0);
  return EULER_OK;
}

static inline int loc_red_blocks(const euler_sim* S) { return (int)eu_blocks(S->e_cnt, EU_RED_ELEMS, 2048); }

int eu_launch_dot(euler_sim* S, const double* a, const double* b, int fin_op, int force) {
  if (S->cfg.dot_mode == EULER_DOT_SEQUENTIAL && !S->has_comm) {
    LAUNCH(S, KC_DOT, k_dot_sequential, dim3(1), dim3(256), a, b, S->cellmask, S->geom, S->sc, fin_op, force);
    return EULER_OK;
  }
  const int edges = (a == S->z && S->has_comm && eu_p2p_has_neighbour_arrays(S)) ? ((S->band_lo > 0 ? 1 : 0) | (S->band_hi < S->geom.nbands ? 2 : 0)) : 0;
  LAUNCH(S, KC_DOT, edges ? k_dot_partial<true> : k_dot_partial<false>, dim3(loc_red_blocks(S)), dim3(RED_THREADS), LOC(a), LOC(b), LOC(S->cellmask), S->e_cnt,
         S->partial, S->sc, force, S->red_counter, fin_or_comm(S, fin_op), edges ? S->geom.TS : 0, edges ? S->band_hi - S->band_lo : 0, edges);
  return S->has_comm ? eu_comm_finish(S, fin_op, 0, force) : EULER_OK;
}

bool tile_recompute(const euler_sim* S) {
  if (S->opt[EULER_OPT_TILE_STORE_AS] || sa_run(S) != 8) return false;
  if (!tile_fused(S)) return !S->has_comm && S->cfg.dot_mode != EULER_DOT_SEQUENTIAL;
  if (S->tile_w != 16) return false;
  if (S->has_comm) return ghost_mode(S);
  return S->cfg.dot_mode != EULER_DOT_SEQUENTIAL;
}
static bool tile_z_begin(euler_sim* S) {
  S->z_halo_last = 0;
  if (!tile_z_recompute(S)) return false;
  if (!S->zhalo) {
    const size_t nh = (size_t)S->geom.nbands * (S->geom.T / 16) * 128, nr = (size_t)S->geom.nbands * 2 * S->X;
    if (eu_dalloc(S, &S->zhalo, nh, EU_MEM_HANDLE, EU_DEV_QUIET)) return false;
    if (eu_dalloc(S, &S->zrows, nr, EU_MEM_HANDLE, EU_DEV_QUIET)) { (void)eu_dev_free(S, S->zhalo); S->zhalo = nullptr; return false; }
    HIPCHK(hipMemsetAsync(S->zhalo, 0, nh * sizeof(double), S->stream));
    HIPCHK(hipMemsetAsync(S->zrows, 0, nr * sizeof(double), S->stream));
  }
  return true;
}

int eu_comm_halo_two(euler_sim* S, double* a, double* b) {
  if (S->p2p_on) { int rc = eu_p2p_halo_skewed(S, a); return rc ? rc : eu_p2p_halo_skewed(S, b); }
  const int X = S->X, nbk = (X + 255) / 256;
  double *send_lo = S->halo_buf, *send_hi = S->halo_buf + 2 * X, *recv_lo = S->halo_buf + 4 * X, *recv_hi = S->halo_buf + 6 * X;
  const int has_lo = S->band_lo > 0, has_hi = S->band_hi < S->geom.nbands;
  hipLaunchKernelGGL(k_halo_rows2<true>, dim3(nbk, 4), dim3(256), 0, S->stream, a, b, send_lo, send_hi, S->geom, S->band_lo, S->band_hi, has_lo, has_hi);
  COMM_CALL(S->comm.halo(S->comm.ctx, send_lo, send_hi, recv_lo, recv_hi, 2 * X));
  hipLaunchKernelGGL(k_halo_rows2<false>, dim3(nbk, 4), dim3(256), 0, S->stream, a, b, recv_lo, recv_hi, S->geom, S->band_lo, S->band_hi, has_lo, has_hi);
  return EULER_OK;
}

static inline bool dot_rides_in_sweep(const euler_sim* S) { return S->cfg.precond == EULER_PRECOND_IC0 && S->cfg.sweep_mode != EULER_SWEEP_SIMPLE && !S->has_comm && S->cfg.dot_mode != EULER_DOT_SEQUENTIAL; }
static int launch_precondition(euler_sim* S, int force, int fin_dot = -1) {
  if (S->cfg.precond == EULER_PRECOND_JACOBI) {
    LAUNCH(S, KC_JACOBI, k_jacobi, dim3(eu_blocks(S->e_cnt, 256 * 4, 4096)), dim3(256), LOC(S->r), LOC(S->z), LOC(S->cellmask),
           S->e_cnt, S->sc, force);
    return fin_dot >= 0 ? eu_launch_dot(S, S->z, S->r, fin_dot, force) : EULER_OK;
  }
  const bool ride = fin_dot >= 0 && dot_rides_in_sweep(S);
  int rc = eu_launch_sweep(S, SW_FORWARD, KC_FORWARD_SOLVE, force, ride ? fin_dot : -1);
  if (rc) return rc;
  if ((rc = eu_launch_sweep(S, SW_BACKWARD, KC_BACKWARD_SOLVE, force))) return rc;
  return fin_dot >= 0 && !ride ? eu_launch_dot(S, S->z, S->r, fin_dot, force) : EULER_OK;
}

static int launch_apply_a_and_alpha(euler_sim* S, int force) {
  const bool seq = S->cfg.dot_mode == EULER_DOT_SEQUENTIAL && !S->has_comm;
  if (S->has_comm && ghost_mode(S) && !force) {
    const int X = S->X, nbk = (X + 255) / 256;
    const bool coarse = eu_is_two_level(S);
    if (S->band_lo > 0) {
      HIPCHK(hipMemcpyAsync(xrow(S, XR_GS_LO0), xrow(S, XR_ZRECV_LO), (size_t)X * 8, hipMemcpyDeviceToDevice, S->stream));
      if (coarse) { int rc = eu_launch_coarse_add_row(S, xrow(S, XR_GS_LO0), 64 * S->band_lo - 1); if (rc) return rc; }
      hipLaunchKernelGGL(k_unpack_row, dim3(nbk), dim3(256), 0, S->stream, S->s, xrow(S, XR_GS_LO0), S->geom, S->band_lo - 1, 63);
    }
    if (S->band_hi < S->geom.nbands) {
      HIPCHK(hipMemcpyAsync(xrow(S, XR_GS_HI0), xrow(S, XR_ZRECV_HI), (size_t)X * 8, hipMemcpyDeviceToDevice, S->stream));
      if (coarse) { int rc = eu_launch_coarse_add_row(S, xrow(S, XR_GS_HI0), 64 * S->band_hi); if (rc) return rc; }
      hipLaunchKernelGGL(k_unpack_row, dim3(nbk), dim3(256), 0, S->stream, S->s, xrow(S, XR_GS_HI0), S->geom, S->band_hi, 0);
    }
    S->gs_cur = 0;
  } else if (S->has_comm) { int rc = comm_halo_s(S); if (rc) return rc; }
  SkewGeom gl = S->geom;
  gl.S = S->e_cnt;
  double* out = tile_fused(S) ? S->q : S->z;
  LAUNCH(S, KC_APPLY_A, k_apply_a, dim3(loc_red_blocks(S)), dim3(RED_THREADS), LOC(S->s), LOC(out), LOC(S->cellmask), gl,
         S->partial, S->sc, force, S->red_counter, seq ? -1 : fin_or_comm(S, FIN_ALPHA));
  if (seq)
    LAUNCH(S, KC_DOT, k_dot_sequential, dim3(1), dim3(256), out, S->s, S->cellmask, S->geom, S->sc, (int)FIN_ALPHA, force);
  return S->has_comm ? eu_comm_finish(S, FIN_ALPHA, 0, force) : EULER_OK;
}

int p_steps(const euler_sim* S) {
  if (S->p2p_on || sa_run(S) != 8) return 2;
  return (int)S->opt[EULER_OPT_P_STEPS];
}
static int ring_begin(euler_sim* S) {
  const int n = p_steps(S);
  if (!S->s_base[0]) { S->s_base[0] = S->s; S->s_base[1] = S->s2; }
  if (n > 2) { S->s = S->s_base[0]; S->s2 = S->s_base[1]; }
  else if (S->s != S->s_base[0] && S->s != S->s_base[1]) { S->s = S->s_base[0]; S->s2 = S->s_base[1]; }
  else if (S->s2 != S->s_base[0] && S->s2 != S->s_base[1]) S->s2 = S->s == S->s_base[0] ? S->s_base[1] : S->s_base[0];
  S->s_ring[0] = S->s; S->s_ring[1] = S->s2;
  for (int k = 2; k < n; ++k) {
    if (!S->s_ring_alloc[k]) {
      const size_t elems = S->Sw + EU_SKEW_SLACK;
      if (eu_dev_alloc(S, &S->s_ring_alloc[k], elems * sizeof(double), EU_MEM_RING, EU_DEV_QUIET)) {
        eu_dev_free_group(S, EU_MEM_RING);
        for (void*& d : S->s_ring_alloc) d = nullptr;
        S->opt[EULER_OPT_P_STEPS] = 2;
        return ring_begin(S);
      }
      HIPCHK(hipMemsetAsync(S->s_ring_alloc[k], 0, elems * sizeof(double), S->stream));
    }
    S->s_ring[k] = static_cast<double*>(S->s_ring_alloc[k]) + EU_SKEW_SLACK - S->skew_off;
  }
  S->s_ring_n = n;
  S->s_launched = 0;
  return EULER_OK;
}
double* eu_current_search_direction(euler_sim* S) {
  if (S->s_ring_n < 2 || S->s_launched <= 0) return S->s;
  (void)hipStreamSynchronize(S->stream);
  const int ran = S->sc_host->nonzero ? S->sc_host->iters : 0;
  if (ran <= 0 || ran > S->s_launched) return S->s;
  return S->s_ring[(ran - 1) % S->s_ring_n];
}

__global__ void k_pcg_reset(PcgScalars* sc, double tol, int max_iters) {
  sc->sigma = sc->zs = sc->sigma_new = sc->alpha = sc->alpha_prev = sc->beta = sc->rnorm = 0.0;
  sc->tol = tol; sc->nonzero = 0; sc->done = 0; sc->iters = 0; sc->max_iters = max_iters; sc->zfix = 0;
}

static inline bool first_direction_folded(const euler_sim* S) { return tile_fused(S) && eu_is_mg(S) && !S->has_comm && S->cfg.dot_mode != EULER_DOT_SEQUENTIAL && sa_run(S) == 8; }
struct Solve {
  PcgScalars prev;
  int pred_iters;
  bool drain_poll;
  bool zr, zr_ran;
  bool solved;
};

static int project_begin(euler_sim* S, float dt, Solve& v) {
  S->s_launched = 0;
  S->z_halo_last = 0;
  S->pcg_fields_resident = 0;
  v.prev = *S->sc_host;
  S->solve_iters[S->solve_seq & 255] = S->sc_host->nonzero ? S->sc_host->iters : -1;
  if (S->solve_seq > 0) { S->res_last_chunks = S->sc_host->n_chunks; S->res_have_last = 1; }
  S->solve_seq += 1;
  v.pred_iters = (S->sc_host->nonzero && S->sc_host->done && S->sc_host->iters < S->cfg.max_iterations) ? S->sc_host->iters : 0;
  v.drain_poll = S->p2p_on && !(S->sc_host->nonzero && !S->sc_host->done && S->sc_host->iters >= S->cfg.max_iterations);
  S->prof_iter = -1;
  LAUNCH(S, KC_MISC, k_pcg_reset, dim3(1), dim3(1), S->sc, S->cfg.tol, S->cfg.max_iterations);
  eu_launch_build_system(S, dt);
  if (S->has_comm) {
    hipLaunchKernelGGL(k_nonzero_to_comm, dim3(1), dim3(1), 0, S->stream, S->sc);
    COMM_CALL(S->comm.allreduce(S->comm.ctx, &S->sc->comm_val, 1, 1));
    hipLaunchKernelGGL(k_nonzero_from_comm, dim3(1), dim3(1), 0, S->stream, S->sc);
  }
  return EULER_OK;
}

static int project_resident(euler_sim* S, float dt, Solve& v) {
  const bool res_skip = S->res_skip_once != 0;
  S->res_skip_once = 0;
  if (!res_skip && eu_resident_eligible(S)) {
    const unsigned int cap_chunks = 4u * (unsigned int)eu_resident_capacity(S, S->cfg.pcg_precision == EULER_PCG_F32);
    unsigned int guess = S->res_last_chunks;
    if (!S->res_have_last) {
      HIPCHK(hipMemcpyAsync(S->sc_host, S->sc, sizeof(PcgScalars), hipMemcpyDeviceToHost, S->stream));
      HIPCHK(hipStreamSynchronize(S->stream));
      guess = S->sc_host->n_chunks;
    }
    if (guess + guess / 16 + 8 <= cap_chunks || S->cfg.pcg_precision == EULER_PCG_F32) {
      v.solved = true;
      S->prof_iter = -2;
      if (int rc = eu_launch_resident(S, cap_chunks)) return rc;
      HIPCHK(hipMemcpyAsync(S->sc_host, S->sc, sizeof(PcgScalars), hipMemcpyDeviceToHost, S->stream));
      HIPCHK(hipStreamSynchronize(S->stream));
      S->res_last_chunks = S->sc_host->n_chunks; S->res_have_last = 1;
      const int err = *S->res_err;
      if (err == 0) {
        if (S->sc_host->nonzero) { S->res_solves += 1; S->pcg_fields_resident = 1; }
        return eu_launch_velocity_update(S, dt, 0);
      }
      *S->res_err = 0;
      if (S->cfg.pcg_precision == EULER_PCG_F32 && err == 2) { eu_set_error("EULER_PCG_F32: the solve's active chunks do not fit the resident solver"); return EULER_EHIP; }
      if (err != 2) { S->res_fallbacks += 1; S->res_disabled = 1; }
      S->solve_seq -= 1;
      eu_vd_solver_arrays_foreign(&S->vd);
      S->res_skip_once = 1;
      *S->sc_host = v.prev;
      return eu_launch_project(S, dt);
    }
  }
  return EULER_OK;
}

static int project_first_direction(euler_sim* S, Solve& v) {
  int rc;
  const bool tile = tile_fused(S), two_level = tile && eu_is_two_level(S);
  if (two_level && S->has_comm && !(eu_is_mg(S) && ghost_mode(S) && S->slab_on)) {
    eu_set_error("coarse-correction preconditioners with several ranks: EULER_PRECOND_IC0_TILE_MG on row slabs without mailboxes only");
    return EULER_EINVAL;
  }
  if (two_level && (rc = eu_launch_coarse_setup(S))) return rc;
  if (two_level && (rc = eu_launch_coarse_consistent(S))) return rc;
  v.zr = tile && tile_z_begin(S);
  if (tile) {
    if ((rc = eu_launch_factor_tile(S, 0))) return rc;
    if ((rc = eu_launch_precond_tile(S, 0, 1, FIN_SIGMA_INIT, 0, 0.0))) return rc;
  } else {
  if (S->cfg.precond != EULER_PRECOND_JACOBI && (rc = eu_launch_sweep(S, SW_FACTOR, KC_PRECON_FACTOR, 0))) return rc;
  if ((rc = launch_precondition(S, 0, FIN_SIGMA_INIT))) return rc;
  }
  if ((rc = ring_begin(S))) return rc;
  if (first_direction_folded(S)) {
    const PcgScalars& ps = v.prev;
    if (ps.nonzero && !(std::isfinite(ps.alpha) && std::isfinite(ps.beta) && std::isfinite(ps.rnorm) && std::isfinite(ps.sigma) && std::isfinite(ps.zs)))
      for (int k = 0; k < S->s_ring_n; ++k) HIPCHK(hipMemsetAsync(S->s_ring[k] + S->skew_off, 0, S->Sw * sizeof(double), S->stream));
  }
  else if (two_level) { if ((rc = eu_launch_coarse_search_init(S))) return rc; }
  else
  LAUNCH(S, KC_UPDATE_SEARCH, k_update_search<true>, dim3(eu_blocks(S->e_cnt, 256 * 4, 4096)), dim3(256), LOC(S->s), LOC(S->z),
         LOC(S->cellmask), S->e_cnt, S->sc, 0, 0.0);
  if (S->has_comm && eu_p2p_has_neighbour_arrays(S)) {
    const int y0 = S->band_lo > 0 ? 64 * S->band_lo : -1, y1 = S->band_hi < S->geom.nbands ? 64 * S->band_hi - 1 : -1;
    LAUNCH(S, KC_UPDATE_SEARCH, k_publish_edge_rows, dim3((S->X + 255) / 256, 2), dim3(256), S->s, S->geom, y0, y1, S->sc);
  }
  if (S->s_ring_n == 2) HIPCHK(hipMemsetAsync(LOC(S->s2), 0, S->e_cnt * sizeof(double), S->stream));
  S->s_stale = 1;
  return EULER_OK;
}

static int project_iterate(euler_sim* S, Solve& v) {
  int rc;
  HIPCHK(hipMemcpyAsync(S->sc_host, S->sc, sizeof(PcgScalars), hipMemcpyDeviceToHost, S->stream));
  HIPCHK(hipStreamSynchronize(S->stream));
  const int poll = S->cfg.pcg_poll_interval > 0 ? S->cfg.pcg_poll_interval : 8;
  const int max_it = S->cfg.max_iterations;
  const bool tile = tile_fused(S), fold0 = first_direction_folded(S);
  int it = 0, chunk = 0;
  bool stop = !S->sc_host->nonzero;
  S->s_none = stop ? 1 : 0;
  while (it < max_it && !stop) {
    int chunk_end = it + poll;
    if (!v.drain_poll && v.pred_iters > 0 && it < v.pred_iters + poll && chunk_end > v.pred_iters - 2) {
      const int lo = v.pred_iters - 2 < chunk_end ? v.pred_iters - 2 : chunk_end;
      chunk_end = lo > it + 2 ? lo : it + 2;
    }
    if (chunk_end > max_it) chunk_end = max_it;
    for (; it < chunk_end; ++it) {
      S->prof_iter = it;
      const bool fused = it > 0 || fold0;
      if (it == 0 && fold0) { S->s = S->s_ring[S->s_ring_n - 1]; S->s2 = S->s_ring[0]; }
      if ((rc = fused ? eu_launch_search_apply(S, it) : launch_apply_a_and_alpha(S, 0))) return rc;
      if (tile) {
        S->prof_iter = it;
        const int nx = it + 1, steps = S->s_ring_n;
        const bool next_odd = !(nx >= steps && nx % steps == 0);
        const int zform = v.zr && it + 1 < max_it ? (it + 2 < max_it && next_odd ? 1 : 0) : -1;
        if ((rc = eu_launch_precond_tile(S, 1, it + 1 < max_it, FIN_BETA, 0, 0.0, false, zform))) return rc;
        S->z_halo_last = zform == 1;
        v.zr_ran = v.zr_ran || zform == 1;
        continue;
      }
      S->tile_as_override = fused ? S->q : S->z;
      rc = eu_launch_precond_tile(S, 1, 0, -1, 0, 0.0, true);
      S->tile_as_override = nullptr;
      if (rc) return rc;
      if (it + 1 < max_it) {
        S->prof_iter = it + 1;
        if ((rc = launch_precondition(S, 0, FIN_BETA))) return rc;
      }
    }
    if (it < max_it && v.drain_poll) {
      HIPCHK(hipMemcpyAsync(S->sc_host, S->sc, sizeof(PcgScalars), hipMemcpyDeviceToHost, S->stream));
      HIPCHK(hipStreamSynchronize(S->stream));
      stop = S->sc_host->done != 0;
    } else
    if (it < max_it) {
      const int slot = chunk & 1;
      if (chunk > 0) {
        HIPCHK(hipEventSynchronize(S->poll_event[slot ^ 1]));
        stop = S->poll_host[slot ^ 1].done != 0;
      }
      HIPCHK(hipMemcpyAsync(&S->poll_host[slot], S->sc, sizeof(PcgScalars), hipMemcpyDeviceToHost, S->stream));
      HIPCHK(hipEventRecord(S->poll_event[slot], S->stream));
      ++chunk;
    }
  }
  return EULER_OK;
}

static int project_finish(euler_sim* S, float dt, const Solve& v) {
  int rc;
  S->prof_iter = -2;
  S->z_halo_last = 0;
  if (v.zr_ran && (rc = eu_launch_precond_tile(S, 0, 1, -1, 0, 0.0, false, 2))) return rc;
  const bool finish_in_update = !S->has_comm && !S->slab_on && S->opt[EULER_OPT_VELOCITY_TWO_PASS] == 0;
  if (!finish_in_update) { if ((rc = eu_launch_finish_p(S))) return rc; }
  if (S->s_ring_n > 2) { S->s = S->s_base[0]; S->s2 = S->s_base[1]; }
  if (S->has_comm && S->slab_on) {
    const int X = S->X, nbk = (X + 255) / 256;
    double *send_lo = S->halo_buf, *send_hi = S->halo_buf + X, *recv_lo = S->halo_buf + 2 * X, *recv_hi = S->halo_buf + 3 * X;
    if (S->band_lo > 0) hipLaunchKernelGGL(k_pack_row, dim3(nbk), dim3(256), 0, S->stream, S->p, send_lo, S->geom, S->band_lo, 0);
    COMM_CALL(S->bulk.halo(S->bulk.ctx, send_lo, send_hi, recv_lo, recv_hi, X));
    if (S->band_hi < S->geom.nbands) hipLaunchKernelGGL(k_unpack_row, dim3(nbk), dim3(256), 0, S->stream, S->p, recv_hi, S->geom, S->band_hi, 0);
  } else if (S->has_comm) {
    const int n = S->comm.nranks, nb = S->geom.nbands;
    std::vector<int64_t> off(n), cnt(n);
    for (int k = 0; k < n; ++k) {
      const int64_t lo = (int64_t)nb * k / n, hi = (int64_t)nb * (k + 1) / n;
      off[k] = lo * S->geom.TS * 64 * 8;
      cnt[k] = (hi - lo) * S->geom.TS * 64 * 8;
    }
    COMM_CALL(S->comm.allgather(S->comm.ctx, S->p, off.data(), cnt.data()));
  }
  if ((rc = eu_launch_velocity_update(S, dt, finish_in_update ? 1 : 0))) return rc;
  HIPCHK(hipMemcpyAsync(S->sc_host, S->sc, sizeof(PcgScalars), hipMemcpyDeviceToHost, S->stream));
  return EULER_OK;
}

int eu_launch_project(euler_sim* S, float dt) {
  Solve v = {};
  int rc;
  if ((rc = project_begin(S, dt, v))) return rc;
  if ((rc = project_resident(S, dt, v)) || v.solved) return rc;
  if ((rc = project_first_direction(S, v))) return rc;
  if ((rc = project_iterate(S, v))) return rc;
  return project_finish(S, dt, v);
}

int eu_launch_pcg_op(euler_sim* S, int op, float dt, double a, double* out) {
  S->s_none = 0;
  S->s_launched = 0;
  const bool want_scalar = op == EULER_OP_DOT_ZR || op == EULER_OP_DOT_ZS || op == EULER_OP_INF_NORM_R;
  const size_t SS = S->geom.S;
  if (eu_is_two_level(S) && (op == EULER_OP_PRECON_FACTOR || op == EULER_OP_FORWARD_SOLVE || op == EULER_OP_BACKWARD_SOLVE)) {
    eu_set_error("euler_pcg_op: the preconditioner of EULER_PRECOND_IC0_TILE2 / _MG is not available as a single operation (select EULER_PRECOND_IC0_TILE for its tile level)");
    return EULER_EINVAL;
  }
  switch (op) {
    case EULER_OP_BUILD_SYSTEM:
      LAUNCH(S, KC_MISC, k_pcg_reset, dim3(1), dim3(1), S->sc, S->cfg.tol, S->cfg.max_iterations);
      eu_launch_build_system(S, dt);
      break;
    case EULER_OP_PRECON_FACTOR: if (tile_fused(S)) eu_launch_factor_tile(S, 1); else eu_launch_sweep(S, SW_FACTOR, KC_PRECON_FACTOR, 1); break;
    case EULER_OP_FORWARD_SOLVE: if (!tile_fused(S)) eu_launch_sweep(S, SW_FORWARD, KC_FORWARD_SOLVE, 1); break;
    case EULER_OP_BACKWARD_SOLVE:
      if (tile_fused(S)) eu_launch_precond_tile(S, 0, 1, FIN_STORE_ONLY, 1, 0.0); else eu_launch_sweep(S, SW_BACKWARD, KC_BACKWARD_SOLVE, 1);
      break;
    case EULER_OP_APPLY_A:
      LAUNCH(S, KC_APPLY_A, k_apply_a, dim3(S->red_blocks), dim3(RED_THREADS), S->s, S->z, S->cellmask, S->geom,
             S->partial, S->sc, 1, S->red_counter, -1);
      break;
    case EULER_OP_DOT_ZR: eu_launch_dot(S, S->z, S->r, FIN_STORE_ONLY, 1); break;
    case EULER_OP_DOT_ZS: eu_launch_dot(S, S->z, S->s, FIN_STORE_ONLY, 1); break;
    case EULER_OP_INF_NORM_R:
      LAUNCH(S, KC_UPDATE_PR, k_inf_norm, dim3(S->red_blocks), dim3(RED_THREADS), S->r, S->cellmask, SS, S->partial);
      LAUNCH(S, KC_REDUCE_FINAL, k_reduce_final<true>, dim3(1), dim3(RED_THREADS), S->partial, S->red_blocks, S->sc,
             (int)FIN_STORE_ONLY, 1);
      break;
    case EULER_OP_UPDATE_PR:
      LAUNCH(S, KC_UPDATE_PR, k_update_pr, dim3(S->red_blocks), dim3(RED_THREADS), S->p, S->r, S->s, S->z, S->cellmask,
             SS, S->partial, S->sc, 1, a, S->red_counter, -1);
      break;
    case EULER_OP_UPDATE_SEARCH:
      LAUNCH(S, KC_UPDATE_SEARCH, k_update_search<false>, dim3(eu_blocks(SS, 256 * 4, 4096)), dim3(256), S->s, S->z,
             S->cellmask, SS, S->sc, 1, a);
      break;
    default: eu_set_error("unknown pcg op %d", op); return EULER_EINVAL;
  }
  HIPCHK(hipMemcpyAsync(S->sc_host, S->sc, sizeof(PcgScalars), hipMemcpyDeviceToHost, S->stream));
  HIPCHK(hipStreamSynchronize(S->stream));
  if (want_scalar && out) *out = S->sc_host->sigma_new;
  return EULER_OK;
}
```

### euler_amd/csrc/k_search.hip

```cpp
#include "k_pcg.h"

#include <type_traits>

#define SA_THREADS 256
struct SaPair { sw_d2 z, so; double ez0, es0, ez1, es1; };

__device__ __forceinline__ double pick3(int t, int tb1, int tb2, double v0, double v1, double v2) {
  double v = v0;
  v = t >= tb1 ? v1 : v;
  v = t >= tb2 ? v2 : v;
  return v;
}
template <int SLAB, int PMODE, int SA_RUN, int COARSE = 0, bool STORE = true, bool ZR = false>
__global__ __launch_bounds__(SA_THREADS, (COARSE == 2 && PMODE == 1 && SLAB == 0) ? 4 : 1) void k_search_apply(const double* __restrict__ s_old, const double* __restrict__ z,
                                                             double* __restrict__ s_new, double* __restrict__ out,
                                                             const uint8_t* __restrict__ mask, SkewGeom g,
                                                             double* __restrict__ partial, PcgScalars* sc, int force,
                                                             unsigned int* counter, int fin_op, SlabNeighbours nbr,
                                                             double* __restrict__ p, double* s_new_base, double* s_old_base,
                                                             const unsigned int* __restrict__ chunk_list,
                                                             CoarseRef cref, SaHist hist, ZrArgs zr) {
  static_assert(PMODE == 1 || PMODE == 2 || PMODE == 4 || PMODE == 8, "PMODE: p is left alone (1) or takes the N fmadds that are due (the ring's length)");
  static_assert(!ZR || (SLAB == 0 && SA_RUN == 8 && COARSE == 0), "ZR: one GPU, runs of one tile, no coarse part");
  __shared__ double s_cy[COARSE == 2 ? SA_THREADS / 64 : 1][COARSE == 2 ? MG_NI + 1 : 1][64];
  __shared__ double s_ce[COARSE == 2 ? SA_THREADS / 64 : 1][COARSE == 2 ? MG_NI + 1 : 1][64];
  if (!force && pcg_idle(sc)) return;
  __shared__ sw_d2 s_ztab[ZR ? 8 : 1][64];
  if (ZR) {
    for (int k = threadIdx.x; k < 8 * 64; k += SA_THREADS) (&s_ztab[0][0])[k] = reinterpret_cast<const sw_d2*>(zr.table)[k];
    __syncthreads();
  }
  const double beta = sc->beta;
  (void)s_new_base; (void)s_old_base;
  constexpr int NPA = PMODE >= 2 ? PMODE : 2;
  double al[NPA] = {};
  if (PMODE >= 2) {
    const int k = sc->iters;
#pragma unroll
    for (int j = 0; j < NPA; ++j) al[j] = sc->alpha_hist[(k - NPA + j) & 7];
  }
  const int lane = threadIdx.x & 63;
  const int TS = g.TS, npairs = TS / 2;
  const int nb_local = (int)(g.S / ((size_t)TS * 64));
  const int cpb = (npairs + SA_RUN - 1) / SA_RUN, total = nb_local * cpb;
  const int n_waves = gridDim.x * (SA_THREADS / 64);
  const bool edge_lane = lane == 0 || lane == 63;
  double t = 0.0;
  const bool listed = chunk_list != nullptr;
  const int ntb16 = g.T / 16;
  const int todo = listed ? (int)sc->n_chunks : total;
  typedef std::integral_constant<bool, true> yes_t;
  typedef std::integral_constant<bool, false> no_t;
  for (int i = blockIdx.x * (SA_THREADS / 64) + (threadIdx.x >> 6); i < todo; i += n_waves) {
    int c = i, per = cpb;
    bool interior = false;
    if (listed) { const unsigned int ent = chunk_list[i]; interior = (ent & EU_CHUNK_INTERIOR) != 0; c = (int)(ent & ~EU_CHUNK_INTERIOR); per = ntb16; }
    const int lb = c / per, P0 = (c % per) * SA_RUN, P1 = ZR ? P0 + SA_RUN : (P0 + SA_RUN < npairs ? P0 + SA_RUN : npairs);
    const size_t bbase = (size_t)lb * TS * 64 + 2 * lane;
    auto run = [&](auto full_tag) {
      constexpr bool FULL = decltype(full_tag)::value;
      unsigned int mm[SA_RUN];
      unsigned int any = 0;
#pragma unroll
      for (int j = 0; j < SA_RUN; ++j) {
        if (FULL) mm[j] = CM_INTERIOR | (CM_INTERIOR << 8);
        else mm[j] = P0 + j < P1 ? (unsigned int)*reinterpret_cast<const unsigned short*>(mask + bbase + (size_t)(P0 + j) * 128) : 0u;
        any |= mm[j];
      }
      if (!FULL && !listed && !__ballot(((any | (any >> 8)) & CM_FLUID) != 0)) return;
      sw_d2 zz[ZR ? SA_RUN : 1];
      if (ZR) {
        sw_d2 rr[SA_RUN], pp[SA_RUN];
#pragma unroll
        for (int j = 0; j < SA_RUN; ++j) {
          rr[j] = *reinterpret_cast<const sw_d2*>(zr.r + bbase + (size_t)(P0 + j) * 128);
          pp[j] = FULL ? s_ztab[j][lane] : *reinterpret_cast<const sw_d2*>(zr.pre + bbase + (size_t)(P0 + j) * 128);
        }
        double none = 0.0;
        tile_solve<2 * SA_RUN, false>(mm, rr, pp, zz, none);
      }
      const int ztile = P0 / SA_RUN;
      const bool up_remote = SLAB == 1 && nbr.z_up && lb + 1 == nb_local, dn_remote = SLAB == 1 && nbr.z_dn && lb == 0;
      const double* ez = lane == 0 ? (dn_remote ? nbr.z_dn : z) : (up_remote ? nbr.z_up : z);
      const double* es = lane == 0 ? (dn_remote ? nbr.s_dn : s_old) : (up_remote ? nbr.s_up : s_old);
      const bool remote = lane == 0 ? dn_remote : up_remote;
      const long long e0_base = lane == 0 ? ((long long)(lb - 1) * TS + 62) * 64 + 127 : ((long long)(lb + 1) * TS - 64) * 64 + 1;
      const long long e1_base = lane == 0 ? ((long long)(lb - 1) * TS + 64) * 64 + 126 : ((long long)(lb + 1) * TS - 62) * 64;
      const unsigned int vbit = lane == 0 ? CM_DOWN : CM_UP;
      const bool ghost = SLAB == 2 && (lane == 0 ? (nbr.zrow_dn != nullptr && lb == 0) : (nbr.zrow_up != nullptr && lb + 1 == nb_local));
      const double* gz = lane == 0 ? nbr.zrow_dn : nbr.zrow_up;
      const double* gs = lane == 0 ? nbr.srow_dn : nbr.srow_up;
      double* gsn = lane == 0 ? nbr.snew_dn : nbr.snew_up;
      const int gcol = lane == 0 ? 0 : -63;
      const double* zrow = ZR ? zr.rows + (long long)(lane == 0 ? 2 * lb - 1 : 2 * lb + 2) * zr.X : nullptr;
      double cy0 = 0.0, cy1 = 0.0, cy2 = 0.0, ce0 = 0.0, ce1 = 0.0, ce2 = 0.0;
      double (*cyv)[64] = s_cy[COARSE == 2 ? threadIdx.x >> 6 : 0];
      double (*cev)[64] = s_ce[COARSE == 2 ? threadIdx.x >> 6 : 0];
      int ctb1 = 0x7fffffff, ctb2 = 0x7fffffff, cJb = 0;
      (void)cJb;
      if (COARSE == 2) {
        cJb = (2 * (P0 - 1) - lane - MG_G0 / 2) >> MG_LOG;
        ctb1 = MG_G0 * (cJb + 1) + lane + MG_G0 / 2;
        const int row = (cref.band0 + lb) * 64 + lane;
        const int hi_ = cref.nx - 1;
        int i0, i1;
        double fy;
        mg_cell_w(row, cref.ny, i0, i1, fy);
        const double* y0 = cref.y + (size_t)i0 * cref.nx;
        const double* y1 = cref.y + (size_t)i1 * cref.nx;
#pragma unroll
        for (int q = 0; q <= MG_NI; ++q) { const int c = cJb + q < 0 ? 0 : (cJb + q < hi_ ? cJb + q : hi_); cyv[q][lane] = mg_rows(y0[c], y1[c], fy); }
#pragma unroll
        for (int q = 0; q <= MG_NI; ++q) cev[q][lane] = 0.0;
        if (edge_lane) {
          const int re = row + (lane == 0 ? -1 : 1);
          if (re >= 0 && re < MG_G0 * cref.ny) {
            mg_cell_w(re, cref.ny, i0, i1, fy);
            y0 = cref.y + (size_t)i0 * cref.nx; y1 = cref.y + (size_t)i1 * cref.nx;
#pragma unroll
            for (int q = 0; q <= MG_NI; ++q) { const int c = cJb + q < 0 ? 0 : (cJb + q < hi_ ? cJb + q : hi_); cev[q][lane] = mg_rows(y0[c], y1[c], fy); }
          }
        }
// ... 113 lines not shown
              v = v - ((m0 & CM_UP) ? up0 : 0.0);
              v = v - ((m0 & CM_LEFT) ? prev_y : 0.0);
              v = v - ((m0 & CM_DOWN) ? dn0 : 0.0);
              o.x = v;
              t += v * cc.x;
            }
            if (m1 & CM_FLUID) {
              double v = (double)(int)(m1 >> CM_DIAG_SHIFT) * cc.y;
              v = v - ((m1 & CM_RIGHT) ? nxt.x : 0.0);
              v = v - ((m1 & CM_UP) ? up1 : 0.0);
              v = v - ((m1 & CM_LEFT) ? cc.x : 0.0);
              v = v - ((m1 & CM_DOWN) ? dn1 : 0.0);
              o.y = v;
              t += v * cc.y;
            }
            if ((m0 & m1) & CM_FLUID) *reinterpret_cast<sw_d2*>(s_new + i) = cc;
            else if (m0 & CM_FLUID) s_new[i] = cc.x;
            else s_new[i + 1] = cc.y;
            if (STORE) {
              if ((m0 & m1) & CM_FLUID) *reinterpret_cast<sw_d2*>(out + i) = o;
              else if (m0 & CM_FLUID) out[i] = o.x;
              else out[i + 1] = o.y;
            }
            if (SLAB == 1 && slab_edge_row(i, lane, TS, nb_local, (nbr.z_dn ? 1 : 0) | (nbr.z_up ? 2 : 0))) {
              if (m0 & CM_FLUID) st_system(s_new + i, cc.x);
              if (m1 & CM_FLUID) st_system(s_new + i + 1, cc.y);
            }
          }
          prev_y = cur.y; cur = nxt;
          B = Cn; Cn = D;
        }
      }
    };
    if (SA_RUN == 8 && interior) run(yes_t()); else run(no_t());
  }
  if (SLAB == 1) asm volatile("s_waitcnt vmcnt(0)" ::: "memory");
  t = block_sum<SA_THREADS>(t);
  if (fin_op >= 0) block_finish<false, SA_THREADS>(t, partial, counter, sc, fin_op);
}

static inline unsigned sa_blocks(const euler_sim* S, int run) {
  return eu_blocks((size_t)(S->band_hi - S->band_lo) * ((S->geom.TS / 2 + run - 1) / run), SA_THREADS / 64, 2048);
}
struct SaCall { SkewGeom gl; int fin; SlabNeighbours nbr; CoarseRef cref; SaHist hist; ZrArgs zr; };
template <int SLAB, int PMODE, int RUN, int COARSE, bool STORE, bool ZR = false>
static void sa_launch(euler_sim* S, const SaCall& c) {
  LAUNCH(S, KC_APPLY_A, (k_search_apply<SLAB, PMODE, RUN, COARSE, STORE, ZR>), dim3(sa_blocks(S, RUN)), dim3(SA_THREADS), LOC(S->s), LOC(S->z), LOC(S->s2),
         LOC(S->q), LOC(S->cellmask), c.gl, S->partial, S->sc, 0, S->red_counter, c.fin, c.nbr, LOC(S->p), S->s2, S->s, RUN == 8 ? S->chunk_list : (const unsigned int*)nullptr, c.cref, c.hist, c.zr);
}
template <int SLAB, int COARSE, int PMODE>
static void sa_pick_run(euler_sim* S, const SaCall& c, int run, bool store) {
  if constexpr (COARSE == 0 && SLAB != 2 && PMODE <= 2) {
    if constexpr (SLAB == 0) { if (run == 16) return sa_launch<SLAB, PMODE, 16, COARSE, true>(S, c); }
    if (run != 8) return sa_launch<SLAB, PMODE, 32, COARSE, true>(S, c);
  }
  if (store) sa_launch<SLAB, PMODE, 8, COARSE, true>(S, c); else sa_launch<SLAB, PMODE, 8, COARSE, false>(S, c);
}
template <int SLAB, int COARSE>
static void sa_pick(euler_sim* S, const SaCall& c, int pmode, int run, bool store) {
  if constexpr (SLAB != 1) {
    if (pmode == 8) return sa_pick_run<SLAB, COARSE, 8>(S, c, run, store);
    if (pmode == 4) return sa_pick_run<SLAB, COARSE, 4>(S, c, run, store);
  }
  if (pmode == 2) sa_pick_run<SLAB, COARSE, 2>(S, c, run, store); else sa_pick_run<SLAB, COARSE, 1>(S, c, run, store);
}
int eu_launch_search_apply(euler_sim* S, int it) {
  const bool seq = S->cfg.dot_mode == EULER_DOT_SEQUENTIAL && !S->has_comm;
  SlabNeighbours nbr = {nullptr, nullptr, nullptr, nullptr, S->band_hi - S->band_lo, nullptr, nullptr, nullptr, nullptr, nullptr, nullptr};
  const bool direct = S->has_comm && eu_p2p_has_neighbour_arrays(S);
  const bool ghost = ghost_mode(S);
  if (ghost) {
    const int c = S->gs_cur;
    if (S->band_lo > 0) { nbr.zrow_dn = xrow(S, XR_ZRECV_LO); nbr.srow_dn = xrow(S, XR_GS_LO0 + c); nbr.snew_dn = xrow(S, XR_GS_LO0 + (c ^ 1)); }
    if (S->band_hi < S->geom.nbands) { nbr.zrow_up = xrow(S, XR_ZRECV_HI); nbr.srow_up = xrow(S, XR_GS_HI0 + c); nbr.snew_up = xrow(S, XR_GS_HI0 + (c ^ 1)); }
    S->gs_cur = c ^ 1;
  } else if (direct) {
    eu_p2p_neighbour_arrays(S, &nbr.z_dn, &nbr.s_dn, &nbr.z_up, &nbr.s_up);
    if (nbr.z_dn) { nbr.z_dn += S->e_lo; nbr.s_dn += S->e_lo; }
    if (nbr.z_up) { nbr.z_up += S->e_lo; nbr.s_up += S->e_lo; }
  } else if (S->has_comm) {
    if (int rc = eu_comm_halo_two(S, S->z, S->s)) return rc;
  }
  const int steps = S->s_ring_n;
  const int pmode = (it >= steps && it % steps == 0) ? steps : 1;
  const bool mg = eu_is_mg(S);
  SaCall c = {S->geom, S->has_comm ? fin_or_comm(S, FIN_ALPHA) : (seq ? -1 : (int)FIN_ALPHA), nbr,
              {mg ? S->mg_x : S->cc_y, mg ? 0 : S->coarse_shift, mg ? S->mg_nx[0] : S->coarse_nx, mg ? S->mg_ny[0] : S->coarse_ny, S->band_lo},
              {{nullptr, nullptr, nullptr, nullptr, nullptr, nullptr}}, {S->r, S->precon, S->tile_table, S->zhalo, S->zrows, S->X}};
  c.gl.S = S->e_cnt;
  for (int j = 1; j + 1 < steps; ++j) c.hist.s[j - 1] = LOC(S->s_ring[j]);
  const int run = sa_run(S);
  const bool store = !tile_recompute(S);
  const bool coarse = eu_is_two_level(S) && tile_fused(S);
  if (S->z_halo_last) sa_launch<0, 1, 8, 0, false, true>(S, c);
  else if (coarse && ghost) sa_pick<2, 2>(S, c, pmode, run, store);
  else if (coarse && mg) sa_pick<0, 2>(S, c, pmode, run, store);
  else if (coarse) sa_pick<0, 1>(S, c, pmode, run, store);
  else if (ghost) sa_pick<2, 0>(S, c, pmode, run, store);
  else if (direct) sa_pick<1, 0>(S, c, pmode, run, store);
  else sa_pick<0, 0>(S, c, pmode, run, store);
  S->s = S->s_ring[it % steps]; S->s2 = S->s_ring[(it + 1) % steps];
  S->s_launched = it + 1;
  if (seq) eu_launch_dot(S, S->q, S->s, FIN_ALPHA, 0);
  return S->has_comm ? eu_comm_finish(S, FIN_ALPHA, 0, 0) : EULER_OK;
}
```

### euler_amd/csrc/k_tile.hip

```cpp
#include "k_pcg.h"

#include <type_traits>

#define PT_THREADS 256
__device__ __forceinline__ void tile_block_reduce(double& mx, double& sm) {
  __shared__ double s_mx[PT_THREADS / 64], s_sm[PT_THREADS / 64];
  mx = eu_wave_max(mx);
  sm = eu_wave_sum(sm);
  __syncthreads();
  if ((threadIdx.x & 63) == 0) { s_mx[threadIdx.x >> 6] = mx; s_sm[threadIdx.x >> 6] = sm; }
  __syncthreads();
  if (threadIdx.x == 0) {
    mx = s_mx[0]; sm = s_sm[0];
    for (int k = 1; k < PT_THREADS / 64; ++k) { mx = s_mx[k] > mx ? s_mx[k] : mx; sm += s_sm[k]; }
  }
}

__global__ __launch_bounds__(64) void k_tile_table(double* __restrict__ tab) {
  const int lane = threadIdx.x & 63;
  double own = 0.0, out = 0.0;
  sw_d2 pp[8];
#pragma unroll
  for (int j = 0; j < 16; ++j) {
    const double nbv = wave_shift_inject<DPP_WAVE_SHR1>(out, 0.0);
    const double res = factor_step(4.0, own, nbv);
    own = res; out = res;
    if (j & 1) pp[j >> 1].y = res; else pp[j >> 1].x = res;
  }
#pragma unroll
  for (int P = 0; P < 8; ++P) reinterpret_cast<sw_d2*>(tab)[P * 64 + lane] = pp[P];
}
int eu_launch_tile_table(euler_sim* S) {
  hipLaunchKernelGGL(k_tile_table, dim3(1), dim3(64), 0, S->stream, S->tile_table);
  return EULER_OK;
}

template <int W>
__global__ __launch_bounds__(PT_THREADS) void k_factor_tile(TileArgs a) {
  if (!a.force && pcg_idle(a.sc)) return;
  const int lane = threadIdx.x & 63;
  const int ntb = a.g.T / W, total = a.nb_local * ntb;
  const int n_waves = gridDim.x * (PT_THREADS / 64);
  for (int tile = blockIdx.x * (PT_THREADS / 64) + (threadIdx.x >> 6); tile < total; tile += n_waves) {
    const int band = a.band_lo + tile / ntb, k = tile % ntb;
    const size_t base = ((size_t)band * a.g.TS + (size_t)k * W) * 64 + 2 * lane;
    unsigned int mm[W / 2];
    unsigned int any = 0;
#pragma unroll
    for (int P = 0; P < W / 2; ++P) { mm[P] = *reinterpret_cast<const unsigned short*>(a.mask + base + P * 128); any |= mm[P]; }
    if (!__ballot(((any | (any >> 8)) & CM_FLUID) != 0)) continue;
    sw_d2 pp[W / 2];
#pragma unroll
    for (int P = 0; P < W / 2; ++P) pp[P] = *reinterpret_cast<const sw_d2*>(a.pre + base + P * 128);
    double own = 0.0, out = 0.0;
#pragma unroll
    for (int j = 0; j < W; ++j) {
      const int cm = (int)((mm[j >> 1] >> ((j & 1) * 8)) & 0xff);
      const double cpre = (j & 1) ? pp[j >> 1].y : pp[j >> 1].x;
      const double nbv = wave_shift_inject<DPP_WAVE_SHR1>(out, 0.0);
      const double aa = (double)(cm >> CM_DIAG_SHIFT);
      const double res = (cm & CM_FLUID) ? factor_step(aa, own, nbv) : cpre;
      own = res; out = res;
      if (j & 1) pp[j >> 1].y = res; else pp[j >> 1].x = res;
    }
#pragma unroll
    for (int P = 0; P < W / 2; ++P) *reinterpret_cast<sw_d2*>(a.pre + base + P * 128) = pp[P];
  }
}

#ifndef PT_RECOMP_BLOCKS
#define PT_RECOMP_BLOCKS 1
#endif
template <int W, bool RECOMP = false, int CMODE = 0>
__global__ __launch_bounds__(PT_THREADS, RECOMP ? PT_RECOMP_BLOCKS : 1) void k_precond_tile(TileArgs a) {
  if (!a.force && (a.zform == 2 ? a.sc->zfix == 0 : pcg_idle(a.sc))) return;
  const int lane = threadIdx.x & 63;
  const int ntb = a.g.T / W, total = a.nb_local * ntb;
  const int n_waves = gridDim.x * (PT_THREADS / 64);
  const double nalpha = -(a.force ? a.alpha_arg : a.sc->alpha);
  double mx = 0.0, dsum = 0.0;
  const bool listed = W == 16 && a.list != nullptr;
  const int todo = listed ? (int)a.sc->n_chunks : total;
  constexpr int TABP = W == 16 ? 8 : 1;
  __shared__ sw_d2 s_tab[TABP][64];
  __shared__ double s_cpart[CMODE == 2 ? PT_THREADS / 64 : 1][CMODE == 2 ? 16 * 2 * MG_NSLOT : 1];
  (void)s_cpart;
  const bool have_tab = W == 16 && listed && a.table != nullptr;
  if (have_tab) {
    for (int k = threadIdx.x; k < TABP * 64; k += PT_THREADS) (&s_tab[0][0])[k] = reinterpret_cast<const sw_d2*>(a.table)[k];
    __syncthreads();
  }
  typedef std::integral_constant<bool, true> yes_t;
  typedef std::integral_constant<bool, false> no_t;
  for (int i = blockIdx.x * (PT_THREADS / 64) + (threadIdx.x >> 6); i < todo; i += n_waves) {
    const int ii = a.reverse ? todo - 1 - i : i;
    const unsigned int ent = listed ? a.list[ii] : (unsigned int)ii;
    const bool interior = have_tab && (ent & EU_CHUNK_INTERIOR) != 0;
    const int tile = (int)(listed ? ent & ~EU_CHUNK_INTERIOR : ent);
    const int band = a.band_lo + tile / ntb, k = tile % ntb;
    const size_t base = ((size_t)band * a.g.TS + (size_t)k * W) * 64 + 2 * lane;
    auto run = [&](auto full_tag) {
      constexpr bool FULL = decltype(full_tag)::value;
      unsigned int mm[W / 2];
      unsigned int any = 0;
#pragma unroll
      for (int P = 0; P < W / 2; ++P) {
        mm[P] = FULL ? (unsigned int)(CM_INTERIOR | (CM_INTERIOR << 8)) : (unsigned int)*reinterpret_cast<const unsigned short*>(a.mask + base + P * 128);
        any |= mm[P];
      }
      if (!FULL && !listed && !__ballot(((any | (any >> 8)) & CM_FLUID) != 0)) return;
      sw_d2 rr[W / 2], qq[W / 2], pp[W / 2];
#pragma unroll
      for (int P = 0; P < W / 2; ++P) {
        rr[P] = *reinterpret_cast<const sw_d2*>(a.r + base + P * 128);
        if (RECOMP && a.rupd) continue;
        if (!a.sweeps) pp[P] = sw_d2{0.0, 0.0};
        else if (FULL) pp[P] = s_tab[P < TABP ? P : 0][lane];
        else pp[P] = *reinterpret_cast<const sw_d2*>(a.pre + base + P * 128);
        if (!RECOMP && a.rupd) qq[P] = *reinterpret_cast<const sw_d2*>(a.as + base + P * 128);
      }
      if (RECOMP && a.rupd) {
        const int npairs = a.g.TS / 2, P0 = k * (W / 2);
        sw_d2 ss[W / 2 + 2];
#pragma unroll
        for (int P = -1; P <= W / 2; ++P)
          ss[P + 1] = (P0 + P >= 0 && P0 + P < npairs) ? *reinterpret_cast<const sw_d2*>(a.as + base + (long long)P * 128) : sw_d2{0.0, 0.0};
        double ev = 0.0;
        if (lane < 16) {
          const int x = k * W + lane;
          if (x < a.g.X) {
            if (a.gs_lo && band == a.band_lo) ev = a.gs_lo[x];
            else if (band > 0) ev = a.as[skew_index(a.g, x, 64 * band - 1)];
          }
        } else if (lane >= 48) {
          const int x = k * W + lane - 48 - 63;
          if (x >= 0 && x < a.g.X) {
            if (a.gs_hi && band == a.band_lo + a.nb_local - 1) ev = a.gs_hi[x];
            else if (band + 1 < a.g.nbands) ev = a.as[skew_index(a.g, x, 64 * (band + 1))];
          }
        }
        const int ev_lo = __double2loint(ev), ev_hi = __double2hiint(ev);
#pragma unroll
        for (int P = 0; P < W / 2; ++P) {
          const unsigned int m0 = mm[P] & 0xff, m1 = mm[P] >> 8;
          const sw_d2 cc = ss[P + 1];
          const double prev_y = ss[P].y, nxt_x = ss[P + 2].x;
          const double d0 = __hiloint2double(__builtin_amdgcn_readlane(ev_hi, 2 * P), __builtin_amdgcn_readlane(ev_lo, 2 * P));
          const double d1 = __hiloint2double(__builtin_amdgcn_readlane(ev_hi, 2 * P + 1), __builtin_amdgcn_readlane(ev_lo, 2 * P + 1));
          const double u0 = __hiloint2double(__builtin_amdgcn_readlane(ev_hi, 48 + 2 * P), __builtin_amdgcn_readlane(ev_lo, 48 + 2 * P));
          const double u1 = __hiloint2double(__builtin_amdgcn_readlane(ev_hi, 49 + 2 * P), __builtin_amdgcn_readlane(ev_lo, 49 + 2 * P));
          const double dn0 = wave_shift_inject<DPP_WAVE_SHR1>(prev_y, d0), up0 = wave_shift_inject<DPP_WAVE_SHL1>(cc.y, u0);
          const double dn1 = wave_shift_inject<DPP_WAVE_SHR1>(cc.x, d1), up1 = wave_shift_inject<DPP_WAVE_SHL1>(nxt_x, u1);
          double v = (double)(int)(m0 >> CM_DIAG_SHIFT) * cc.x;
          v = v - ((m0 & CM_RIGHT) ? cc.y : 0.0);
          v = v - ((m0 & CM_UP) ? up0 : 0.0);
          v = v - ((m0 & CM_LEFT) ? prev_y : 0.0);
          v = v - ((m0 & CM_DOWN) ? dn0 : 0.0);
          if (m0 & CM_FLUID) { rr[P].x = rr[P].x + v * nalpha; const double w = fabs(rr[P].x); if (w > mx) mx = w; }
// ... 29 lines not shown
#pragma unroll
        for (int j = 0; j < W; ++j) {
          const int cm = (int)((mm[j >> 1] >> ((j & 1) * 8)) & 0xff);
          const double rv = (cm & CM_FLUID) ? ((j & 1) ? rr[j >> 1].y : rr[j >> 1].x) : 0.0;
          const double jv = rv * (double)j;
#pragma unroll
          for (int m = 0; m < MG_NSEG; ++m) {
            const bool in = (m == 0 || j >= tbase + MG_G0 * m) && (m == MG_NSEG - 1 || j < tbase + MG_G0 * (m + 1));
            sg_s[m] += in ? rv : 0.0; sg_t[m] += in ? jv : 0.0;
          }
        }
        double cn[MG_NSEG + 1];
#pragma unroll
        for (int m = 0; m <= MG_NSEG; ++m) cn[m] = 0.0;
#pragma unroll
        for (int m = 0; m < MG_NSEG; ++m) {
          double u1 = sg_t[m] + (double)(-tbase - MG_G0 * m) * sg_s[m], u0 = (double)MG_G0 * sg_s[m] - u1;
          if (Jb + m < 0) { u0 = 0.0; u1 = (double)MG_G0 * sg_s[m]; }
          if (Jb + m >= a.cnx - 1) { u0 = (double)MG_G0 * sg_s[m]; u1 = 0.0; }
          cn[m] += u0; cn[m + 1] += u1;
        }
        const bool shifted = Jb != Jq;
        wy0 *= 1.0 / (MG_G0 * MG_G0); wy1 *= 1.0 / (MG_G0 * MG_G0);
        double* sp = s_cpart[threadIdx.x >> 6];
#pragma unroll
        for (int q = 0; q < MG_NSLOT; ++q) {
          const double lo = cn[q], hi = q >= 1 ? cn[q - 1] : 0.0;
          const double cs = shifted ? hi : lo;
          const double p0 = group_sum(wy0 * cs), p1 = group_sum(wy1 * cs);
          if ((lane & 3) == 0) { sp[quad * 2 * MG_NSLOT + q] = p0; sp[quad * 2 * MG_NSLOT + MG_NSLOT + q] = p1; }
        }
        __builtin_amdgcn_fence(__ATOMIC_RELEASE, "wavefront");
        __builtin_amdgcn_wave_barrier();
        {
          double* cp = a.cpart + ((size_t)(tile / ntb) * MG_NGRP * ntb + (size_t)k) * (2 * MG_NSLOT);
#pragma unroll
          for (int u = 0; u < (MG_PART + 63) / 64; ++u) {
            const int e = lane + 64 * u;
            if (e < MG_PART) {
              const int g = e / (2 * MG_NSLOT), w = e % (2 * MG_NSLOT);
              const double va = g > 0 ? sp[(2 * g - 1) * 2 * MG_NSLOT + w] : 0.0, vb = g < 8 ? sp[(2 * g) * 2 * MG_NSLOT + w] : 0.0;
              cp[((size_t)g * ntb) * (2 * MG_NSLOT) + w] = va + vb;
            }
          }
        }
        __builtin_amdgcn_fence(__ATOMIC_ACQUIRE, "wavefront");
        __builtin_amdgcn_wave_barrier();
      } else if (W == 16 && CMODE == 1) {
        const int xl = k * W - 63, J0 = (xl > 0 ? xl : 0) >> a.cshift;
        double c0 = 0.0, c1 = 0.0, c2 = 0.0;
#pragma unroll
        for (int j = 0; j < W; ++j) {
          const int cm = (int)((mm[j >> 1] >> ((j & 1) * 8)) & 0xff);
          const double rv = (cm & CM_FLUID) ? ((j & 1) ? rr[j >> 1].y : rr[j >> 1].x) : 0.0;
          const int x = k * W + j - lane;
          const int b = ((x > 0 ? x : 0) >> a.cshift) - J0;
          c0 += b == 0 ? rv : 0.0; c1 += b == 1 ? rv : 0.0; c2 += b == 2 ? rv : 0.0;
        }
        c0 = eu_wave_sum(c0); c1 = eu_wave_sum(c1); c2 = eu_wave_sum(c2);
        if (lane == 0) { double* cp = a.cpart + (size_t)tile * 3; cp[0] = c0; cp[1] = c1; cp[2] = c2; }
      }
      if (RECOMP && a.rupd) {
        asm volatile("" ::: "memory");
#pragma unroll
        for (int P = 0; P < W / 2; ++P) pp[P] = FULL ? s_tab[P < TABP ? P : 0][lane] : *reinterpret_cast<const sw_d2*>(a.pre + base + P * 128);
      }
      tile_solve<W, true>(mm, rr, pp, qq, dsum);
      if (W == 16 && a.zform == 1) {
        double* h = a.zhalo + ((size_t)band * ntb + k) * 128;
        h[lane] = qq[0].x;
        h[64 + lane] = qq[W / 2 - 1].y;
        if (lane == 0 || lane == 63) {
          double* row = a.zrows + ((size_t)band * 2 + (lane == 63 ? 1 : 0)) * a.g.X;
#pragma unroll
          for (int j = 0; j < W; ++j) {
            const int x = k * W + j - lane;
            if (x >= 0 && x < a.g.X) row[x] = (j & 1) ? qq[j >> 1].y : qq[j >> 1].x;
          }
        }
      } else {
#pragma unroll
        for (int P = 0; P < W / 2; ++P) *reinterpret_cast<sw_d2*>(a.z + base + P * 128) = qq[P];
      }
      if (band == a.edge_lo || band == a.edge_hi) {
        const bool lo = band == a.edge_lo && lane == 0, hi = band == a.edge_hi && lane == 63;
#pragma unroll
        for (int j = 0; j < W; ++j) {
          const double zv = (j & 1) ? qq[j >> 1].y : qq[j >> 1].x;
          const int x_lo = k * W + j, x_hi = k * W + j - 63;
          if (lo && x_lo < a.g.X) a.zsend_lo[x_lo] = zv;
          if (hi && x_hi >= 0 && x_hi < a.g.X) a.zsend_hi[x_hi] = zv;
        }
      }
    };
    if (W == 16 && interior) run(yes_t()); else run(no_t());
  }
  tile_block_reduce(mx, dsum);
  __shared__ int am_last;
  if (threadIdx.x == 0) {
    __hip_atomic_store(reinterpret_cast<unsigned long long*>(&a.part_max[blockIdx.x]), (unsigned long long)__double_as_longlong(mx), __ATOMIC_RELAXED, __HIP_MEMORY_SCOPE_AGENT);
    __hip_atomic_store(reinterpret_cast<unsigned long long*>(&a.part_dot[blockIdx.x]), (unsigned long long)__double_as_longlong(dsum), __ATOMIC_RELAXED, __HIP_MEMORY_SCOPE_AGENT);
    asm volatile("s_waitcnt vmcnt(0)" ::: "memory");
    const unsigned int t = __hip_atomic_fetch_add(a.counter, 1u, __ATOMIC_RELAXED, __HIP_MEMORY_SCOPE_AGENT);
    am_last = t == gridDim.x - 1;
  }
  __syncthreads();
  if (!am_last) return;
  double vmax = 0.0, vsum = 0.0;
  for (unsigned int i = threadIdx.x; i < gridDim.x; i += PT_THREADS) {
    const double m = __longlong_as_double((long long)__hip_atomic_load(reinterpret_cast<unsigned long long*>(&a.part_max[i]), __ATOMIC_RELAXED, __HIP_MEMORY_SCOPE_AGENT));
    const double d = __longlong_as_double((long long)__hip_atomic_load(reinterpret_cast<unsigned long long*>(&a.part_dot[i]), __ATOMIC_RELAXED, __HIP_MEMORY_SCOPE_AGENT));
    vmax = m > vmax ? m : vmax; vsum += d;
  }
  tile_block_reduce(vmax, vsum);
  if (a.via == FIN_VIA_P2P) {
    if (a.rupd) vmax = p2p_allreduce_block<true>(a.sc, vmax);
    if (a.fin_dot >= 0) vsum = p2p_allreduce_block<false>(a.sc, vsum);
  }
  if (threadIdx.x == 0) {
    if (a.via == FIN_TO_COMM) { a.pair_slot[0] = vmax; a.pair_slot[1] = vsum; }
    else {
      if (a.rupd) pcg_scalar_step(a.sc, FIN_RNORM, vmax);
      if (a.fin_dot >= 0 && !(a.rupd && a.sc->done)) pcg_scalar_step(a.sc, a.fin_dot, vsum);
    }
    if (a.zform >= 0) a.sc->zfix = a.zform == 1 ? 1u : 0u;
    __hip_atomic_store(a.counter, 0u, __ATOMIC_RELAXED, __HIP_MEMORY_SCOPE_AGENT);
  }
}

__global__ void k_pair_fold(PcgScalars* sc, const double* __restrict__ pairs, int stride, int R, int rupd, int fin_dot, int force) {
  if (!force && pcg_idle(sc)) return;
  double vmax = 0.0, vsum = 0.0;
  for (int r = 0; r < R; ++r) { vmax = pairs[(size_t)stride * r] > vmax ? pairs[(size_t)stride * r] : vmax; vsum += pairs[(size_t)stride * r + 1]; }
  if (rupd) pcg_scalar_step(sc, FIN_RNORM, vmax);
  if (fin_dot >= 0 && !(rupd && sc->done)) pcg_scalar_step(sc, fin_dot, vsum);
}
static TileArgs make_tile_args(euler_sim* S, int force) {
  TileArgs a;
  a.g = S->geom; a.mask = S->cellmask; a.pre = S->precon; a.r = S->r; a.as = S->tile_as_override ? S->tile_as_override : S->q; a.z = S->z;
  a.band_lo = S->band_lo; a.nb_local = S->band_hi - S->band_lo;
  a.rupd = 0; a.sweeps = 1; a.fin_dot = -1;
  a.via = S->has_comm ? (S->p2p_on ? (int)FIN_VIA_P2P : (int)FIN_TO_COMM) : 0;
  a.part_max = S->partial; a.part_dot = S->partial2; a.counter = S->red_counter; a.sc = S->sc; a.force = force; a.alpha_arg = 0.0;
  a.pair_slot = S->pair_buf + 2 * (S->has_comm ? S->comm.rank : 0);
  a.list = !force ? S->chunk_list : nullptr;
  a.table = S->tile_table;
  a.zsend_lo = a.zsend_hi = nullptr; a.edge_lo = a.edge_hi = -1;
  a.reverse = S->opt[EULER_OPT_TILE_REVERSE] != 0;
  a.cpart = nullptr; a.cshift = 0; a.cmode = 0; a.cnx = a.cny = 0;
  a.gs_lo = a.gs_hi = nullptr;
  a.zform = -1; a.zhalo = S->zhalo; a.zrows = S->zrows;
  if (ghost_mode(S)) {
    if (S->band_lo > 0) { a.zsend_lo = xrow(S, XR_ZSEND_LO); a.edge_lo = S->band_lo; }
    if (S->band_hi < S->geom.nbands) { a.zsend_hi = xrow(S, XR_ZSEND_HI); a.edge_hi = S->band_hi - 1; }
  }
  return a;
}
static inline unsigned tile_blocks(const euler_sim* S, int w) {
  return eu_blocks((size_t)(S->band_hi - S->band_lo) * (S->geom.T / w), PT_THREADS / 64, 2048);
}
typedef void (*TileKernel)(TileArgs);
int eu_launch_factor_tile(euler_sim* S, int force) {
  const TileKernel k = S->tile_w == 8 ? k_factor_tile<8> : S->tile_w == 32 ? k_factor_tile<32> : k_factor_tile<16>;
  LAUNCH(S, KC_PRECON_FACTOR, k, dim3(tile_blocks(S, S->tile_w)), dim3(PT_THREADS), make_tile_args(S, force));
  return EULER_OK;
}
int eu_launch_precond_tile(euler_sim* S, int rupd, int sweeps, int fin_dot, int force, double alpha, bool r_only, int zform) {
  const bool seq = S->cfg.dot_mode == EULER_DOT_SEQUENTIAL && !S->has_comm;
  TileArgs a = make_tile_args(S, force);
  a.rupd = rupd; a.sweeps = sweeps; a.fin_dot = (seq || !sweeps) ? -1 : fin_dot; a.alpha_arg = alpha;
  a.zform = zform;
  const bool two_level = eu_is_two_level(S) && sweeps && !r_only && !force && a.list != nullptr;
  const int fin_real = a.fin_dot;
  if (two_level) {
    const bool mg = eu_is_mg(S);
    a.cpart = mg ? S->mg_part : S->cc_part; a.cshift = mg ? 0 : S->coarse_shift;
    a.cmode = mg ? 2 : 1; a.cnx = mg ? S->mg_nx[0] : 0; a.cny = mg ? S->mg_ny[0] : 0;
    if (a.fin_dot >= 0) a.fin_dot = FIN_STORE_ONLY;
  }
  double* xsmall = S->pair_buf;
  int nsmall = 2;
  bool split = false;
  if (two_level && a.via == FIN_TO_COMM) {
    split = eu_is_mg(S) && ghost_mode(S) && eu_mg_split(S);
    nsmall = eu_coarse_comm_slots(S);
    if (nsmall < 0) return EULER_ENOMEM;
    xsmall = S->mg_xbuf;
    a.pair_slot = xsmall + (size_t)S->comm.rank * nsmall;
    if (split) {
      if (a.zsend_lo) a.zsend_lo = eu_mg_split_msg(S, 0);
      if (a.zsend_hi) a.zsend_hi = eu_mg_split_msg(S, 1);
    }
  }
  const int w = r_only ? 16 : S->tile_w, cls = r_only ? KC_UPDATE_PR : zform == 2 ? KC_MISC : KC_PRECOND_TILE;
  const bool recomp = rupd && !force && tile_recompute(S) && (r_only ? S->tile_as_override == S->q : !S->tile_as_override);
  if (recomp) {
    a.as = S->s;
    if (ghost_mode(S)) {
      if (S->band_lo > 0) a.gs_lo = xrow(S, XR_GS_LO0 + S->gs_cur);
      if (S->band_hi < S->geom.nbands) a.gs_hi = xrow(S, XR_GS_HI0 + S->gs_cur);
    }
  }
  const TileKernel k = w == 8 ? k_precond_tile<8> : w == 32 ? k_precond_tile<32>
                     : a.cmode == 2 ? (recomp ? k_precond_tile<16, true, 2> : k_precond_tile<16, false, 2>)
                     : a.cmode == 1 ? (recomp ? k_precond_tile<16, true, 1> : k_precond_tile<16, false, 1>)
                     : (recomp ? k_precond_tile<16, true> : k_precond_tile<16>);
  LAUNCH(S, cls, k, dim3(tile_blocks(S, w)), dim3(PT_THREADS), a);
  if (two_level && a.via != FIN_TO_COMM) { int rc = eu_launch_coarse_solve(S, fin_real, force); if (rc) return rc; }
  if (seq && sweeps && fin_dot >= 0) eu_launch_dot(S, S->z, S->r, fin_dot, force);
  if (a.via == FIN_TO_COMM) {
    const int R = S->comm.nranks;
    const bool rows = ghost_mode(S) && !force;
    int rc = !two_level ? EULER_OK : split ? eu_mg_split_pre(S) : eu_launch_coarse_pre(S, force);
    if (rc) return rc;
    if (split) rc = eu_comm_exchange(S, eu_mg_split_msg(S, 0), eu_mg_split_msg(S, 1), eu_mg_split_msg(S, 2), eu_mg_split_msg(S, 3), eu_mg_split_count(S), xsmall, nsmall);
    else rc = eu_comm_exchange(S, xrow(S, XR_ZSEND_LO), xrow(S, XR_ZSEND_HI), xrow(S, XR_ZRECV_LO), xrow(S, XR_ZRECV_HI), rows ? S->X : 0, xsmall, nsmall);
    if (rc) return rc;
    hipLaunchKernelGGL(k_pair_fold, dim3(1), dim3(1), 0, S->stream, S->sc, xsmall, nsmall, R, rupd, a.fin_dot, force);
    if (split) {
      if ((rc = eu_mg_split_mid(S, fin_real, force, xrow(S, XR_ZRECV_LO), xrow(S, XR_ZRECV_HI)))) return rc;
      if ((rc = eu_comm_exchange(S, nullptr, nullptr, nullptr, nullptr, 0, eu_mg_split_gc(S), 1 + MG_NULL_MAX))) return rc;
      return eu_mg_split_fold(S, fin_real, force);
    }
    if (two_level) { rc = eu_launch_coarse_scatter(S); if (rc) return rc; rc = eu_launch_coarse_solve(S, fin_real, force); if (rc) return rc; }
  }
  return EULER_OK;
}
```

### include/euler.h

```cpp
#ifndef EULER_H
#define EULER_H

#include <stddef.h>
#include <stdint.h>

#ifdef __cplusplus
extern "C" {
#endif

#define EULER_ABI_VERSION 2

enum {
  EULER_OK = 0,
  EULER_EINVAL = -1,
  EULER_ENOMEM = -2,
  EULER_EIO = -3,
  EULER_EHIP = -4,
  EULER_ESTATE = -5,
  EULER_ETIMEOUT = -6,
  EULER_ECOMM = -7
};

enum {
  EULER_DOT_AUTO = 0,
// ... 297 lines not shown
  float    x, y;
  float    path;
  float    age;
  float    wet_time;
  uint32_t substeps;
  uint32_t flags;
  uint32_t reserved;
} euler_tracer;
int euler_tracers_add(euler_sim* sim, const float* xy, size_t n);
int euler_tracers_count(euler_sim* sim, size_t* n);
int euler_tracers_get(euler_sim* sim, size_t first, size_t n, euler_tracer* out, size_t out_bytes);
int euler_tracers_clear(euler_sim* sim);
enum { EULER_TRACER_RASTER_ALL = 1 };
int euler_tracer_raster(euler_sim* sim, int32_t x0, int32_t y0, int32_t x1, int32_t y1, int32_t W, int32_t H,
                        int32_t flags, uint32_t* out, size_t out_bytes);
int euler_tracer_paint(const uint32_t* counts, euler_overview_px* px, int32_t W, int32_t H,
                       const float fg[3], const float* bg );

#define EULER_BODIES_MAX 16
typedef struct euler_body {
  double  x, y;
  double  hz, phase;
  float   vx, vy;
  float   amp_x, amp_y;
  int32_t w, h;
  int32_t reserved[2];
} euler_body;
typedef struct euler_body_state { double px, py; int32_t ox, oy; } euler_body_state;
int euler_body_at(const euler_body* b, double t, int32_t X, int32_t Y, euler_body_state* out);
int euler_set_bodies(euler_sim* sim, const euler_body* bodies, int32_t n);
int euler_get_bodies(euler_sim* sim, euler_body* bodies, int32_t cap, euler_body_state* now, int32_t* n);

typedef struct euler_reseed {
  int32_t thin_above;
  int32_t fill_holes;
  int32_t max_cells;
  int32_t max_fill;
  int32_t reserved[4];
} euler_reseed;
typedef struct euler_reseed_stats { uint64_t removed, added, cells_thinned, deferred; } euler_reseed_stats;
int euler_set_reseed(euler_sim* sim, const euler_reseed* r);
int euler_get_reseed(euler_sim* sim, euler_reseed* r, euler_reseed_stats* stats);

enum { EULER_ENV_ARRIVAL = 1, EULER_ENV_WET = 2, EULER_ENV_SPEED = 4, EULER_ENV_PRESSURE = 8, EULER_ENV_ALL = 15 };
int euler_set_envelope(euler_sim* sim, uint32_t channels);
int euler_get_envelope(euler_sim* sim, uint32_t* channels, uint64_t* substeps);
int euler_envelope_reset(euler_sim* sim);
int euler_envelope_get_field(euler_sim* sim, int32_t channel, float* dst, size_t bytes);
int euler_envelope_set_field(euler_sim* sim, int32_t channel, const float* src, size_t bytes);
typedef struct euler_envelope_px {
  uint32_t cells;
  uint32_t touched;
  uint32_t arrival_min;
  uint32_t arrival_max;
  uint32_t wet_max;
  uint32_t speed2_max;
  uint32_t p_max;
  uint32_t reserved;
} euler_envelope_px;
int euler_envelope_raster(euler_sim* sim, int32_t x0, int32_t y0, int32_t x1, int32_t y1, int32_t W, int32_t H, euler_envelope_px* out, size_t out_bytes);
int euler_envelope_rgb(const euler_envelope_px* px, int32_t W, int32_t H, int32_t channel, double scale, uint8_t* rgb, size_t rgb_bytes);

typedef struct euler_comm_ops {
  void*   ctx;
  int32_t rank, nranks;
  int (*allreduce)(void* ctx, void* dev_f64, int32_t count, int32_t is_max);
  int (*halo)(void* ctx, void* send_lo, void* send_hi, void* recv_lo, void* recv_hi, int32_t count);
  int (*chain)(void* ctx, void* dev_ptr, int64_t nbytes, int32_t src, int32_t dst);
  int (*allgather)(void* ctx, void* dev_base, const int64_t* off, const int64_t* cnt);
  int (*exchange)(void* ctx, void* send_lo, void* send_hi, void* recv_lo, void* recv_hi, int32_t count, void* small, int32_t nsmall);
} euler_comm_ops;

enum {
  EULER_SLAB_EXACT = 1,
  EULER_SLAB_LOCAL = 0
};
int euler_set_comm(euler_sim* sim, const euler_comm_ops* ops, int32_t coupling);

#define EULER_RCCL_ID_BYTES 128
int euler_rccl_unique_id(void* id_out, int32_t cap);
int euler_rccl_version(void);
int euler_set_comm_rccl(euler_sim* sim, const void* unique_id, int32_t id_bytes, int32_t rank, int32_t nranks,
                        int32_t coupling);
enum {
  EULER_OPT_P_STEPS = 1,
  EULER_OPT_TILE_STORE_AS = 2,
  EULER_OPT_TILE_REVERSE = 3,
  EULER_OPT_RESIDENT_CAP = 4,
  EULER_OPT_GRID4_MIN_CELLS = 5,
  EULER_OPT_SLAB_FUSION = 6,
  EULER_OPT_RCCL_SMALL = 7,
  EULER_OPT_RCCL_NO_EXCHANGE = 8,
  EULER_OPT_MARKERS_ROWMAJOR = 9,
  EULER_OPT_SA_RUN = 10,
  EULER_OPT_NO_INTERIOR = 11,
  EULER_OPT_BUILD_GATHER = 12,
  EULER_OPT_RESIDENT_FORCE_TIMEOUT = 13,
  EULER_OPT_MG_SPLIT_LEVEL = 14,
  EULER_OPT_MG_SPLIT_ACTIVE = 15,
  EULER_OPT_MARKERS_TWO_PASS = 16,
  EULER_OPT_BUILD_TWO_PASS = 17,
  EULER_OPT_VELOCITY_TWO_PASS = 18,
  EULER_OPT_NO_TILE_MAP = 19,
  EULER_OPT_PROFILE_STRIDE = 20,
  EULER_OPT_TILE_STORE_Z = 21,
  EULER_OPT_ADVECT_RK2 = 22,
  EULER_OPT_ADVECT_MACCORMACK = 23,
  EULER_OPT__COUNT
};
int euler_set_option(euler_sim* sim, int32_t key, int64_t value);
int euler_get_option(euler_sim* sim, int32_t key, int64_t* value);

int euler_comm_calls(euler_sim* sim, uint64_t out[5]);

#define EULER_P2P_HANDLE_BYTES 256
int euler_p2p_export(euler_sim* sim, void* handle_out, int32_t cap);
int euler_p2p_connect(euler_sim* sim, const void* handles, int32_t nranks);
int euler_p2p_disconnect(euler_sim* sim);
int euler_p2p_calls(euler_sim* sim, uint64_t out[2]);
int euler_set_stream(euler_sim* sim, void* hip_stream);
int euler_slab_info(euler_sim* sim, int32_t* band_lo, int32_t* band_hi, int32_t* nbands);

int euler_profile_enable(euler_sim* sim, uint64_t class_mask);
int euler_profile_class_count(void);
const char* euler_profile_class_name(int32_t cls);
int euler_profile_get(euler_sim* sim, int32_t cls, double* total_ms, uint64_t* launches);
int euler_profile_reset(euler_sim* sim);
int euler_measure_copy_bandwidth(euler_sim* sim, size_t bytes, int32_t reps, double* gbps);
int euler_measure_exchange(euler_sim* sim, int32_t reps, int32_t row_doubles, int32_t nsmall, double* us_per_exchange);
int euler_device_name(euler_sim* sim, char* out, int32_t cap);
uint64_t euler_hbm_bytes(const euler_sim* sim);
int euler_sweep_timeline(euler_sim* sim, uint64_t* out, int32_t cap_bands);

#ifdef __cplusplus
}
#endif
#endif
```

Before: 198.4 million.

## Fold deferred p updates into tile r-update kernel and write first search direction directly

When the tile-local recompute path runs with 8-step p accumulation, the pressure vector's ring of search directions is applied inside the preconditioner r-update kernel every 8 iterations (PFLUSH), and search_apply no longer does the periodic full p flush. The first preconditioner writes z straight into the search direction, which lets the initial k_update_search copy and the apply_A store be skipped. A p_terms counter tracks how many terms are already folded, so finish_p and velocity_update only add the remainder. The intent is to cut separate memory passes over p and z. The cost is a heavier tile kernel, with nine extra vector reads and a p write on flush iterations.

New measurement: 195.3 million. -1.5%, worse.

```diff
diff --git a/euler_amd/__init__.py b/euler_amd/__init__.py
--- a/euler_amd/__init__.py
+++ b/euler_amd/__init__.py
@@ -11,6 +11,7 @@
 (OPT_P_STEPS, OPT_TILE_STORE_AS, OPT_TILE_REVERSE, OPT_RESIDENT_CAP, OPT_GRID4_MIN_CELLS, OPT_SLAB_FUSION, OPT_RCCL_SMALL, OPT_RCCL_NO_EXCHANGE, OPT_MARKERS_ROWMAJOR,
  OPT_SA_RUN, OPT_NO_INTERIOR, OPT_BUILD_GATHER, OPT_RESIDENT_FORCE_TIMEOUT, OPT_MG_SPLIT_LEVEL, OPT_MG_SPLIT_ACTIVE, OPT_MARKERS_TWO_PASS, OPT_BUILD_TWO_PASS,
  OPT_VELOCITY_TWO_PASS, OPT_NO_TILE_MAP, OPT_PROFILE_STRIDE, OPT_TILE_STORE_Z, OPT_ADVECT_RK2, OPT_ADVECT_MACCORMACK) = range(1, 24)
+TILE_Z_P_IN_SEARCH = 2
 SWEEP_AUTO, SWEEP_BAND, SWEEP_SIMPLE = 0, 1, 2
 PCG_F64, PCG_F32 = 0, 1
 RESIDENT_AUTO, RESIDENT_OFF = 0, 1
diff --git a/euler_amd/csrc/driver.hip b/euler_amd/csrc/driver.hip
--- a/euler_amd/csrc/driver.hip
+++ b/euler_amd/csrc/driver.hip
@@ -162,6 +162,7 @@
     case EULER_OPT_MG_SPLIT_LEVEL: ok = value >= -1 && value < 12; break;
     case EULER_OPT_PROFILE_STRIDE: ok = value >= 1 && value <= 1024; break;
     case EULER_OPT_MG_SPLIT_ACTIVE: ok = false; break;
+    case EULER_OPT_TILE_STORE_Z: ok = value >= 0 && value <= EULER_TILE_Z_P_IN_SEARCH; break;
     case EULER_OPT_ADVECT_RK2: ok = value == 0 || value == 1;
       if (ok && value == 1 && S->slab_on) when = "on a whole-grid handle (row slabs: the midpoint samples reach one row beyond the ghost rows)";
       break;
diff --git a/euler_amd/csrc/euler_dev.h b/euler_amd/csrc/euler_dev.h
--- a/euler_amd/csrc/euler_dev.h
+++ b/euler_amd/csrc/euler_dev.h
@@ -43,6 +43,7 @@
   int max_iters;
   unsigned int n_chunks;
   unsigned int zfix;
+  int p_terms;
   void** p2p_boxes;
   int* p2p_error;
   int p2p_rank, p2p_n;
@@ -222,6 +223,7 @@
   int s_none;
   int s_stale;
   const double* tile_as_override;
+  double* tile_z_override;
   double* partial2;
   struct RngJump* rng_jump;
   uint8_t* chunk_flag;
@@ -231,6 +233,7 @@
   double* zhalo;
   double* zrows;
   int z_halo_last;
+  int p_in_rupd;
   double* tile_table;
   unsigned long long* chunk_bits;
   unsigned int* chunk_list;
diff --git a/euler_amd/csrc/k_grid.hip b/euler_amd/csrc/k_grid.hip
--- a/euler_amd/csrc/k_grid.hip
+++ b/euler_amd/csrc/k_grid.hip
@@ -697,7 +697,7 @@
   }
 }
 
-struct VuRing { const double* s[8]; int n, steps, use; };
+struct VuRing { const double* s[8]; int n, use; };
 #define VU_W 48
 #define VU_ILP 4
 __global__ __launch_bounds__(256) void k_velocity_update_para(const float* __restrict__ uin, const float* __restrict__ vin, float* __restrict__ uout, float* __restrict__ vout,
@@ -714,9 +714,8 @@
   if (skip_zero && tmap && eu_tiles_idle_cur(tmap, tnx, band, t0 > 63 ? (t0 - 63) >> 6 : 0, (t0 + VU_W - 1) >> 6, true)) return;
   int cnt = 0, from = 0;
   if (ring.use && sc->nonzero && sc->iters > 0) {
-    const int n_it = sc->iters;
-    from = n_it - 1 >= ring.steps ? (n_it - 1) / ring.steps * ring.steps : 0;
-    cnt = n_it - from;
+    from = sc->p_terms;
+    cnt = sc->iters - from;
   }
   double al[8];
   const double* sq[8];
@@ -906,7 +905,7 @@
   if (one_pass) {
     VuRing ring;
     for (int k = 0; k < 8; ++k) ring.s[k] = S->s_ring[k < S->s_ring_n ? k : 0];
-    ring.n = S->s_ring_n > 0 ? S->s_ring_n : 1; ring.steps = ring.n; ring.use = finish && S->s_ring_n > 0;
+    ring.n = S->s_ring_n > 0 ? S->s_ring_n : 1; ring.use = finish && S->s_ring_n > 0;
     if (!ring.use) for (int k = 0; k < 8; ++k) ring.s[k] = S->p;
     const int do_max = S->slab_on ? 0 : 1;
     if (eu_vd_update_clears_maxima(&S->vd, do_max)) HIPCHK(hipMemsetAsync(&S->ms->max_u2_bits, 0, 2 * sizeof(unsigned int), S->stream));
diff --git a/euler_amd/csrc/k_pcg.h b/euler_amd/csrc/k_pcg.h
--- a/euler_amd/csrc/k_pcg.h
+++ b/euler_amd/csrc/k_pcg.h
@@ -12,7 +12,7 @@
 int eu_launch_band_ranges(euler_sim* S);
 int eu_launch_sweep(euler_sim* S, int op, int cls, int force, int fin_qq = -1);
 int eu_launch_factor_tile(euler_sim* S, int force);
-int eu_launch_precond_tile(euler_sim* S, int rupd, int sweeps, int fin_dot, int force, double alpha, bool r_only = false, int zform = -1);
+int eu_launch_precond_tile(euler_sim* S, int rupd, int sweeps, int fin_dot, int force, double alpha, bool r_only = false, int zform = -1, bool pflush = false);
 int eu_launch_search_apply(euler_sim* S, int it);
 int eu_launch_finish_p(euler_sim* S);
 int eu_launch_dot(euler_sim* S, const double* a, const double* b, int fin_op, int force);
@@ -35,7 +35,10 @@
 }
 static inline bool tile_z_recompute(const euler_sim* S) {
   return tile_recompute(S) && tile_fused(S) && !eu_is_two_level(S) && S->tile_w == 16 && !S->has_comm && !S->slab_on && S->band_lo == 0 &&
-         S->opt[EULER_OPT_TILE_STORE_Z] == 0 && S->chunk_list && S->tile_table;
+         S->opt[EULER_OPT_TILE_STORE_Z] != 1 && S->chunk_list && S->tile_table;
+}
+static inline bool tile_p_in_rupd(const euler_sim* S) {
+  return tile_z_recompute(S) && p_steps(S) == 8 && S->opt[EULER_OPT_TILE_STORE_Z] == 0;
 }
 static inline int fin_or_comm(const euler_sim* S, int fin_op) {
   return S->has_comm ? (S->p2p_on ? (fin_op | FIN_VIA_P2P) : (int)FIN_TO_COMM) : fin_op;
@@ -232,6 +235,8 @@
   const double *gs_lo, *gs_hi;
   int zform;
   double *zhalo, *zrows;
+  double* p;
+  const double* ring[7];
 };
 
 __device__ __forceinline__ double factor_step(double aa, double own, double nbv) {
diff --git a/euler_amd/csrc/k_pcg.hip b/euler_amd/csrc/k_pcg.hip
--- a/euler_amd/csrc/k_pcg.hip
+++ b/euler_amd/csrc/k_pcg.hip
@@ -87,6 +87,7 @@
   if (threadIdx.x == 0) pcg_scalar_step(sc, op, total);
 }
 
+template <bool STORE = true>
 __global__ __launch_bounds__(RED_THREADS) void k_apply_a(const double* __restrict__ s, double* __restrict__ z,
                                                          const uint8_t* __restrict__ mask, SkewGeom g,
                                                          double* __restrict__ partial, PcgScalars* sc, int force,
@@ -145,6 +146,7 @@
       o.y = v;
       t += v * c.y;
     }
+    if (!STORE) continue;
     if ((m0 & m1) & CM_FLUID) *reinterpret_cast<sw_d2*>(z + i) = o;
     else if (m0 & CM_FLUID) z[i] = o.x;
     else z[i + 1] = o.y;
@@ -229,13 +231,14 @@
   }
 }
 
-struct SRing { const double* s[8]; int n, steps; };
+struct SRing { const double* s[8]; int n; };
 __global__ __launch_bounds__(256) void k_finish_p(double* __restrict__ p, const uint8_t* __restrict__ mask, size_t e_lo, size_t S,
                                                   const PcgScalars* sc, SRing ring) {
   if (!sc->nonzero || sc->iters == 0) return;
   const int n_it = sc->iters;
-  const int from = n_it - 1 >= ring.steps ? (n_it - 1) / ring.steps * ring.steps : 0;
+  const int from = sc->p_terms;
   const int cnt = n_it - from;
+  if (cnt <= 0) return;
   double al[8];
   const double* sp[8];
 #pragma unroll
@@ -261,7 +264,7 @@
   if (S->s_ring_n <= 0) return EULER_OK;
   SRing ring;
   for (int k = 0; k < 8; ++k) ring.s[k] = S->s_ring[k < S->s_ring_n ? k : 0];
-  ring.n = S->s_ring_n; ring.steps = S->s_ring_n;
+  ring.n = S->s_ring_n;
   LAUNCH(S, KC_UPDATE_PR, k_finish_p, dim3(eu_blocks(S->e_cnt, 256 * 4, 4096)), dim3(256), S->p + S->e_lo, S->cellmask + S->e_lo, S->e_lo, S->e_cnt, S->sc, ring);
   return EULER_OK;
 }
@@ -399,7 +402,7 @@
   return fin_dot >= 0 && !ride ? eu_launch_dot(S, S->z, S->r, fin_dot, force) : EULER_OK;
 }
 
-static int launch_apply_a_and_alpha(euler_sim* S, int force) {
+static int launch_apply_a_and_alpha(euler_sim* S, int force, bool store = true) {
   const bool seq = S->cfg.dot_mode == EULER_DOT_SEQUENTIAL && !S->has_comm;
   if (S->has_comm && ghost_mode(S) && !force) {
     const int X = S->X, nbk = (X + 255) / 256;
@@ -419,7 +422,7 @@
   SkewGeom gl = S->geom;
   gl.S = S->e_cnt;
   double* out = tile_fused(S) ? S->q : S->z;
-  LAUNCH(S, KC_APPLY_A, k_apply_a, dim3(loc_red_blocks(S)), dim3(RED_THREADS), LOC(S->s), LOC(out), LOC(S->cellmask), gl,
+  LAUNCH(S, KC_APPLY_A, store ? k_apply_a<true> : k_apply_a<false>, dim3(loc_red_blocks(S)), dim3(RED_THREADS), LOC(S->s), LOC(out), LOC(S->cellmask), gl,
          S->partial, S->sc, force, S->red_counter, seq ? -1 : fin_or_comm(S, FIN_ALPHA));
   if (seq)
     LAUNCH(S, KC_DOT, k_dot_sequential, dim3(1), dim3(256), out, S->s, S->cellmask, S->geom, S->sc, (int)FIN_ALPHA, force);
@@ -464,7 +467,7 @@
 
 __global__ void k_pcg_reset(PcgScalars* sc, double tol, int max_iters) {
   sc->sigma = sc->zs = sc->sigma_new = sc->alpha = sc->alpha_prev = sc->beta = sc->rnorm = 0.0;
-  sc->tol = tol; sc->nonzero = 0; sc->done = 0; sc->iters = 0; sc->max_iters = max_iters; sc->zfix = 0;
+  sc->tol = tol; sc->nonzero = 0; sc->done = 0; sc->iters = 0; sc->max_iters = max_iters; sc->zfix = 0; sc->p_terms = 0;
 }
 
 static inline bool first_direction_folded(const euler_sim* S) { return tile_fused(S) && eu_is_mg(S) && !S->has_comm && S->cfg.dot_mode != EULER_DOT_SEQUENTIAL && sa_run(S) == 8; }
@@ -473,12 +476,14 @@
   int pred_iters;
   bool drain_poll;
   bool zr, zr_ran;
+  bool s0_direct;
   bool solved;
 };
 
 static int project_begin(euler_sim* S, float dt, Solve& v) {
   S->s_launched = 0;
   S->z_halo_last = 0;
+  S->p_in_rupd = 0;
   S->pcg_fields_resident = 0;
   v.prev = *S->sc_host;
   S->solve_iters[S->solve_seq & 255] = S->sc_host->nonzero ? S->sc_host->iters : -1;
@@ -543,21 +548,28 @@
   if (two_level && (rc = eu_launch_coarse_setup(S))) return rc;
   if (two_level && (rc = eu_launch_coarse_consistent(S))) return rc;
   v.zr = tile && tile_z_begin(S);
+  const bool ring_first = v.zr && tile_p_in_rupd(S);
+  if (ring_first && (rc = ring_begin(S))) return rc;
+  S->p_in_rupd = ring_first && S->s_ring_n == 8;
+  v.s0_direct = S->p_in_rupd && S->cfg.max_iterations >= 2;
   if (tile) {
     if ((rc = eu_launch_factor_tile(S, 0))) return rc;
-    if ((rc = eu_launch_precond_tile(S, 0, 1, FIN_SIGMA_INIT, 0, 0.0))) return rc;
+    S->tile_z_override = v.s0_direct ? S->s : nullptr;
+    rc = eu_launch_precond_tile(S, 0, 1, FIN_SIGMA_INIT, 0, 0.0);
+    S->tile_z_override = nullptr;
+    if (rc) return rc;
   } else {
   if (S->cfg.precond != EULER_PRECOND_JACOBI && (rc = eu_launch_sweep(S, SW_FACTOR, KC_PRECON_FACTOR, 0))) return rc;
   if ((rc = launch_precondition(S, 0, FIN_SIGMA_INIT))) return rc;
   }
-  if ((rc = ring_begin(S))) return rc;
+  if (!ring_first && (rc = ring_begin(S))) return rc;
   if (first_direction_folded(S)) {
     const PcgScalars& ps = v.prev;
     if (ps.nonzero && !(std::isfinite(ps.alpha) && std::isfinite(ps.beta) && std::isfinite(ps.rnorm) && std::isfinite(ps.sigma) && std::isfinite(ps.zs)))
       for (int k = 0; k < S->s_ring_n; ++k) HIPCHK(hipMemsetAsync(S->s_ring[k] + S->skew_off, 0, S->Sw * sizeof(double), S->stream));
   }
   else if (two_level) { if ((rc = eu_launch_coarse_search_init(S))) return rc; }
-  else
+  else if (!v.s0_direct)
   LAUNCH(S, KC_UPDATE_SEARCH, k_update_search<true>, dim3(eu_blocks(S->e_cnt, 256 * 4, 4096)), dim3(256), LOC(S->s), LOC(S->z),
          LOC(S->cellmask), S->e_cnt, S->sc, 0, 0.0);
   if (S->has_comm && eu_p2p_has_neighbour_arrays(S)) {
@@ -590,13 +602,14 @@
       S->prof_iter = it;
       const bool fused = it > 0 || fold0;
       if (it == 0 && fold0) { S->s = S->s_ring[S->s_ring_n - 1]; S->s2 = S->s_ring[0]; }
-      if ((rc = fused ? eu_launch_search_apply(S, it) : launch_apply_a_and_alpha(S, 0))) return rc;
+      if ((rc = fused ? eu_launch_search_apply(S, it) : launch_apply_a_and_alpha(S, 0, !v.s0_direct))) return rc;
       if (tile) {
         S->prof_iter = it;
         const int nx = it + 1, steps = S->s_ring_n;
-        const bool next_odd = !(nx >= steps && nx % steps == 0);
+        const bool next_odd = S->p_in_rupd || !(nx >= steps && nx % steps == 0);
         const int zform = v.zr && it + 1 < max_it ? (it + 2 < max_it && next_odd ? 1 : 0) : -1;
-        if ((rc = eu_launch_precond_tile(S, 1, it + 1 < max_it, FIN_BETA, 0, 0.0, false, zform))) return rc;
+        const bool pflush = S->p_in_rupd && nx % 8 == 0 && nx < max_it;
+        if ((rc = eu_launch_precond_tile(S, 1, it + 1 < max_it, FIN_BETA, 0, 0.0, false, zform, pflush))) return rc;
         S->z_halo_last = zform == 1;
         v.zr_ran = v.zr_ran || zform == 1;
         continue;
@@ -688,7 +701,7 @@
       if (tile_fused(S)) eu_launch_precond_tile(S, 0, 1, FIN_STORE_ONLY, 1, 0.0); else eu_launch_sweep(S, SW_BACKWARD, KC_BACKWARD_SOLVE, 1);
       break;
     case EULER_OP_APPLY_A:
-      LAUNCH(S, KC_APPLY_A, k_apply_a, dim3(S->red_blocks), dim3(RED_THREADS), S->s, S->z, S->cellmask, S->geom,
+      LAUNCH(S, KC_APPLY_A, k_apply_a<true>, dim3(S->red_blocks), dim3(RED_THREADS), S->s, S->z, S->cellmask, S->geom,
              S->partial, S->sc, 1, S->red_counter, -1);
       break;
     case EULER_OP_DOT_ZR: eu_launch_dot(S, S->z, S->r, FIN_STORE_ONLY, 1); break;
diff --git a/euler_amd/csrc/k_search.hip b/euler_amd/csrc/k_search.hip
--- a/euler_amd/csrc/k_search.hip
+++ b/euler_amd/csrc/k_search.hip
@@ -38,6 +38,7 @@
     const int k = sc->iters;
 #pragma unroll
     for (int j = 0; j < NPA; ++j) al[j] = sc->alpha_hist[(k - NPA + j) & 7];
+    if (blockIdx.x == 0 && threadIdx.x == 0) sc->p_terms = k;
   }
   const int lane = threadIdx.x & 63;
   const int TS = g.TS, npairs = TS / 2;
@@ -317,7 +318,7 @@
     if (int rc = eu_comm_halo_two(S, S->z, S->s)) return rc;
   }
   const int steps = S->s_ring_n;
-  const int pmode = (it >= steps && it % steps == 0) ? steps : 1;
+  const int pmode = (it >= steps && it % steps == 0 && !S->p_in_rupd) ? steps : 1;
   const bool mg = eu_is_mg(S);
   SaCall c = {S->geom, S->has_comm ? fin_or_comm(S, FIN_ALPHA) : (seq ? -1 : (int)FIN_ALPHA), nbr,
               {mg ? S->mg_x : S->cc_y, mg ? 0 : S->coarse_shift, mg ? S->mg_nx[0] : S->coarse_nx, mg ? S->mg_ny[0] : S->coarse_ny, S->band_lo},
diff --git a/euler_amd/csrc/k_tile.hip b/euler_amd/csrc/k_tile.hip
--- a/euler_amd/csrc/k_tile.hip
+++ b/euler_amd/csrc/k_tile.hip
@@ -71,9 +71,16 @@
 #ifndef PT_RECOMP_BLOCKS
 #define PT_RECOMP_BLOCKS 1
 #endif
-template <int W, bool RECOMP = false, int CMODE = 0>
+template <int W, bool RECOMP = false, int CMODE = 0, bool PFLUSH = false>
 __global__ __launch_bounds__(PT_THREADS, RECOMP ? PT_RECOMP_BLOCKS : 1) void k_precond_tile(TileArgs a) {
+  static_assert(!PFLUSH || (W == 16 && RECOMP && CMODE == 0), "PFLUSH: the plain tile-local mode's r update");
   if (!a.force && (a.zform == 2 ? a.sc->zfix == 0 : pcg_idle(a.sc))) return;
+  double al[PFLUSH ? 8 : 1] = {};
+  if (PFLUSH) {
+    const int n_it = a.sc->iters;
+#pragma unroll
+    for (int j = 0; j < 8; ++j) al[j] = a.sc->alpha_hist[(n_it - 8 + j) & 7];
+  }
   const int lane = threadIdx.x & 63;
   const int ntb = a.g.T / W, total = a.nb_local * ntb;
   const int n_waves = gridDim.x * (PT_THREADS / 64);
@@ -269,6 +276,27 @@
 #pragma unroll
         for (int P = 0; P < W / 2; ++P) *reinterpret_cast<sw_d2*>(a.z + base + P * 128) = qq[P];
       }
+      if (PFLUSH) {
+        asm volatile("" ::: "memory");
+#pragma unroll
+        for (int P = 0; P < W / 2; ++P) {
+          const unsigned int m0 = mm[P] & 0xff, m1 = mm[P] >> 8;
+          if ((m0 | m1) & CM_FLUID) {
+            const size_t i = base + P * 128;
+            sw_d2 pv = *reinterpret_cast<const sw_d2*>(a.p + i);
+            sw_d2 sv[8];
+#pragma unroll
+            for (int j = 0; j < 7; ++j) sv[j] = *reinterpret_cast<const sw_d2*>(a.ring[j] + i);
+            sv[7] = *reinterpret_cast<const sw_d2*>(a.as + i);
+#pragma unroll
+            for (int j = 0; j < 8; ++j) {
+              if (m0 & CM_FLUID) pv.x = pv.x + sv[j].x * al[j];
+              if (m1 & CM_FLUID) pv.y = pv.y + sv[j].y * al[j];
+            }
+            *reinterpret_cast<sw_d2*>(a.p + i) = pv;
+          }
+        }
+      }
       if (band == a.edge_lo || band == a.edge_hi) {
         const bool lo = band == a.edge_lo && lane == 0, hi = band == a.edge_hi && lane == 63;
 #pragma unroll
@@ -311,6 +339,7 @@
       if (a.fin_dot >= 0 && !(a.rupd && a.sc->done)) pcg_scalar_step(a.sc, a.fin_dot, vsum);
     }
     if (a.zform >= 0) a.sc->zfix = a.zform == 1 ? 1u : 0u;
+    if (PFLUSH) a.sc->p_terms = a.sc->iters;
     __hip_atomic_store(a.counter, 0u, __ATOMIC_RELAXED, __HIP_MEMORY_SCOPE_AGENT);
   }
 }
@@ -324,7 +353,7 @@
 }
 static TileArgs make_tile_args(euler_sim* S, int force) {
   TileArgs a;
-  a.g = S->geom; a.mask = S->cellmask; a.pre = S->precon; a.r = S->r; a.as = S->tile_as_override ? S->tile_as_override : S->q; a.z = S->z;
+  a.g = S->geom; a.mask = S->cellmask; a.pre = S->precon; a.r = S->r; a.as = S->tile_as_override ? S->tile_as_override : S->q; a.z = S->tile_z_override ? S->tile_z_override : S->z;
   a.band_lo = S->band_lo; a.nb_local = S->band_hi - S->band_lo;
   a.rupd = 0; a.sweeps = 1; a.fin_dot = -1;
   a.via = S->has_comm ? (S->p2p_on ? (int)FIN_VIA_P2P : (int)FIN_TO_COMM) : 0;
@@ -337,6 +366,8 @@
   a.cpart = nullptr; a.cshift = 0; a.cmode = 0; a.cnx = a.cny = 0;
   a.gs_lo = a.gs_hi = nullptr;
   a.zform = -1; a.zhalo = S->zhalo; a.zrows = S->zrows;
+  a.p = nullptr;
+  for (const double*& q : a.ring) q = nullptr;
   if (ghost_mode(S)) {
     if (S->band_lo > 0) { a.zsend_lo = xrow(S, XR_ZSEND_LO); a.edge_lo = S->band_lo; }
     if (S->band_hi < S->geom.nbands) { a.zsend_hi = xrow(S, XR_ZSEND_HI); a.edge_hi = S->band_hi - 1; }
@@ -352,7 +383,7 @@
   LAUNCH(S, KC_PRECON_FACTOR, k, dim3(tile_blocks(S, S->tile_w)), dim3(PT_THREADS), make_tile_args(S, force));
   return EULER_OK;
 }
-int eu_launch_precond_tile(euler_sim* S, int rupd, int sweeps, int fin_dot, int force, double alpha, bool r_only, int zform) {
+int eu_launch_precond_tile(euler_sim* S, int rupd, int sweeps, int fin_dot, int force, double alpha, bool r_only, int zform, bool pflush) {
   const bool seq = S->cfg.dot_mode == EULER_DOT_SEQUENTIAL && !S->has_comm;
   TileArgs a = make_tile_args(S, force);
   a.rupd = rupd; a.sweeps = sweeps; a.fin_dot = (seq || !sweeps) ? -1 : fin_dot; a.alpha_arg = alpha;
@@ -388,7 +419,13 @@
       if (S->band_hi < S->geom.nbands) a.gs_hi = xrow(S, XR_GS_HI0 + S->gs_cur);
     }
   }
-  const TileKernel k = w == 8 ? k_precond_tile<8> : w == 32 ? k_precond_tile<32>
+  if (pflush) {
+    if (!recomp || w != 16 || a.cmode != 0 || !sweeps || S->s_ring_n != 8) { eu_set_error("k_precond_tile: p's ring cannot be applied by this r update"); return EULER_EINVAL; }
+    a.p = S->p;
+    for (int j = 0; j < 7; ++j) a.ring[j] = S->s_ring[j];
+  }
+  const TileKernel k = pflush ? k_precond_tile<16, true, 0, true>
+                     : w == 8 ? k_precond_tile<8> : w == 32 ? k_precond_tile<32>
                      : a.cmode == 2 ? (recomp ? k_precond_tile<16, true, 2> : k_precond_tile<16, false, 2>)
                      : a.cmode == 1 ? (recomp ? k_precond_tile<16, true, 1> : k_precond_tile<16, false, 1>)
                      : (recomp ? k_precond_tile<16, true> : k_precond_tile<16>);
diff --git a/include/euler.h b/include/euler.h
--- a/include/euler.h
+++ b/include/euler.h
@@ -403,6 +403,7 @@
 int euler_rccl_version(void);
 int euler_set_comm_rccl(euler_sim* sim, const void* unique_id, int32_t id_bytes, int32_t rank, int32_t nranks,
                         int32_t coupling);
+#define EULER_TILE_Z_P_IN_SEARCH 2
 enum {
   EULER_OPT_P_STEPS = 1,
   EULER_OPT_TILE_STORE_AS = 2,
```
